# sailordiary/m3f.pytorch

Hardware: AMD Instinct MI355X
Metric: clips/sec (300-frame A+V, fwd+bwd) (higher is better)
Workload: dtype f32 (fp32-accurate products, fp32 accumulate: GEMMs as fp16x3 -- two fp16 terms per scaled operand, three MFMAs, error vs fp64 no larger than an fp32 GEMM's; the forward and backward recurrences at H=512 and H=256 as fp16x3 too (h is bounded; the backward producers split their values under a power-o

## Files before the change

### include/m3t_hip.h

```cpp
#ifndef M3T_HIP_H
#define M3T_HIP_H

#include <stddef.h>
#include <stdint.h>

#ifdef __cplusplus
extern "C" {
#endif

#define M3T_EINVAL 10001
#define M3T_MAX_SCANS 8
#define M3T_ESPIN 10002
#define M3T_SCAN_NO_PERSIST 1
#define M3T_SCAN_WHH 8
#define M3T_SCAN_FP32 4
#define M3T_SCAN_FAULT 16
#define M3T_SCAN_WIDE 32
#define M3T_BF16 2
#define M3T_GEMM_BACKGROUND 1
#define M3T_GEMM_BF16 2
#define M3T_GEMM_HIGH 256
#define M3T_GEMM_F16X3 1024
#define M3T_GEMM_BESIDE_SCAN 512
#define M3T_GEMM_EXCLUSIVE 8
// ... 105 lines not shown
    unsigned long long* amax;
    const float* wfrag;
} m3t_gru_bwd_desc;

size_t m3t_gru_bwd_prepare_floats(int H);
int m3t_gru_bwd_prepare(const float* const* w, int n, int H, int whh_direct, float* const* out, void* stream);

int m3t_gru_scan_workgroups(int n_scans, int H, int B, int T, int flags, int backward);
int m3t_gru_persist_count(void);
int m3t_gru_poll_error(void);
int m3t_gru_error_reset(void);
int m3t_gru_error_defer(int on);
int m3t_gru_inject_error(void* stream);
int m3t_gru_persist_owner(void);
int m3t_gru_scan_arena(void* arena, size_t bytes);
int m3t_gru_scan_arena_reset(void* arena);
int m3t_gru_scan_progress(unsigned* counters, int n_marks, const int* time_bounds, unsigned* need);
int m3t_gru_scan_progress_reset(unsigned* counters);
int m3t_gru_scan_progress_ok(int n_scans, int H, int B, int T, int flags, int backward);
int m3t_stream_wait_progress(const unsigned* counter, unsigned need, void* stream);
int m3t_gru_scan_after(void* event);
int m3t_gru_scan_events(void* start, void* end);
int m3t_gru_persist_profile(unsigned long long* out6);

int m3t_gru_scan_bwd(const m3t_gru_bwd_desc* scans, int n_scans, int B, int T,
                     float* ws, size_t ws_bytes, int flags, void* stream);

int m3t_att_fuse_fwd(const float* s_v, const float* s_a, const float* x_v, const float* x_a,
                     float* f, int rows, int D, void* stream);
int m3t_att_fuse_bwd(const float* df, const float* s_v, const float* s_a,
                     const float* x_v, const float* x_a,
                     float* ds_v, float* ds_a, float* dx_v, float* dx_a,
                     int rows, int D, void* stream);

int m3t_va_loss(const float* y_hat, int rows, int C, int iv, int ia,
                const float* valence, const float* arousal,
                const int64_t* class_expr, const uint8_t* expr_valid, int n_expr,
                float w_v, float w_a, float expr_w, int use_mse,
                float* out_scalars, float* dy, float* ws, size_t ws_bytes, void* stream);
size_t m3t_va_loss_ws_bytes(int rows);

size_t m3t_bn_cl_ws_bytes(size_t M, int C);
int m3t_bn_pool_cl_fwd(const float* x, size_t P, int H, int W, int C, int k, const float* gamma, const float* beta, float* run_mean, float* run_var,
                       float momentum, float eps, int training, float* yp, unsigned char* win, float* save_mean, float* save_invstd, float* ws,
                       size_t ws_bytes, void* stream);
int m3t_bn_pool_cl_bwd(const float* dyp, const float* x, const float* yp, const unsigned char* win, const float* gamma, const float* save_mean,
                       const float* save_invstd, size_t P, int H, int W, int C, int k, int training, float* dx, float* dgamma, float* dbeta,
                       float* dx_colsum, float* ws, size_t ws_bytes, void* stream);
int m3t_bn_cl_fwd(const float* x, size_t M, int C, const float* gamma, const float* beta, float* run_mean, float* run_var, float momentum,
                  float eps, int training, int relu, float* y, float* save_mean, float* save_invstd, float* ws, size_t ws_bytes, void* stream);
int m3t_bn_cl_bwd(const float* dy, const float* x, const float* y, const float* gamma, const float* save_mean, const float* save_invstd, size_t M,
                  int C, int training, int relu, float* dx, float* dgamma, float* dbeta, float* dx_colsum, float* ws, size_t ws_bytes, void* stream);
int m3t_pool_cl_fwd(const float* x, size_t P, int H, int W, int C, int kh, int kw, int sh, int sw, int ph, int pw, float* y, unsigned char* win,
                    void* stream);
int m3t_pool_cl_bwd(const float* dy, const unsigned char* win, size_t P, int H, int W, int C, int kh, int kw, int sh, int sw, int ph, int pw,
                    float* dx, void* stream);

int m3t_bn_add_relu_cl_fwd(const float* x, const float* shortcut, size_t M, int C, const float* gamma, const float* beta, float* run_mean,
                           float* run_var, float momentum, float eps, int training, float* y, float* save_mean, float* save_invstd, float* ws,
                           size_t ws_bytes, void* stream);
int m3t_bn_add_relu_cl_bwd(const float* dy, const float* x, const float* y, const float* gamma, const float* save_mean, const float* save_invstd,
                           size_t M, int C, int training, float* dx, float* ds, float* dgamma, float* dbeta, float* dx_colsum, float* ws,
                           size_t ws_bytes, void* stream);
int m3t_mean_cl_fwd(const float* x, size_t P, int HW, int C, float* y, void* stream);
int m3t_mean_cl_bwd(const float* dy, size_t P, int HW, int C, float* dx, void* stream);

// ... 260 lines not shown
```

### m3f.pytorch_amd/csrc/fuse_loss.hip

```cpp
#include "gru_common.h"
#include <cmath>
#include <cstdlib>
#include <mutex>

namespace {

__device__ __forceinline__ void fuse_weights(float sv, float sa, float& hv, float& ha, float& w0, float& w1) {
    hv = 1.f / (1.f + expf(-sv));
    ha = 1.f / (1.f + expf(-sa));
    const float m = fmaxf(hv, ha);
    const float ev = expf(hv - m), ea = expf(ha - m);
    const float inv = 1.f / (ev + ea);
    w0 = ev * inv;
    w1 = ea * inv;
}

__device__ __forceinline__ float mix2(float w0, float v, float w1, float a) { return fmaf(w0, v, w1 * a); }

__global__ __launch_bounds__(256) void att_fuse_fwd_kernel(const float* __restrict__ s_v, const float* __restrict__ s_a,
                                                           const float* __restrict__ x_v, const float* __restrict__ x_a,
                                                           float* __restrict__ f, int rows, int D, int vec) {
    const int lane = threadIdx.x & 63;
    const int row = blockIdx.x * 4 + (threadIdx.x >> 6);
    if (row >= rows) return;
// ... 23 lines not shown
    if (row >= rows) return;
    float hv, ha, w0, w1;
    fuse_weights(s_v[row], s_a[row], hv, ha, w0, w1);
    const size_t base = (size_t)row * D;
    float d0 = 0.f, d1 = 0.f;
    if (vec) {
        const float4* pg = reinterpret_cast<const float4*>(df + base);
        const float4* pv = reinterpret_cast<const float4*>(x_v + base);
        const float4* pa = reinterpret_cast<const float4*>(x_a + base);
        float4* qv = reinterpret_cast<float4*>(dx_v + base);
        float4* qa = reinterpret_cast<float4*>(dx_a + base);
        for (int i = lane; i < (D >> 2); i += 64) {
            const float4 g = pg[i], v = pv[i], a = pa[i];
            d0 += g.x * v.x + g.y * v.y + g.z * v.z + g.w * v.w;
            d1 += g.x * a.x + g.y * a.y + g.z * a.z + g.w * a.w;
            qv[i] = make_float4(w0 * g.x, w0 * g.y, w0 * g.z, w0 * g.w);
            qa[i] = make_float4(w1 * g.x, w1 * g.y, w1 * g.z, w1 * g.w);
        }
    } else {
        for (int i = lane; i < D; i += 64) {
            const float g = df[base + i];
            d0 += g * x_v[base + i];
            d1 += g * x_a[base + i];
            dx_v[base + i] = w0 * g;
            dx_a[base + i] = w1 * g;
        }
    }
    d0 = wave_sum(d0);
    d1 = wave_sum(d1);
    if (lane == 0) {
        const float dot = w0 * d0 + w1 * d1;
        ds_v[row] = w0 * (d0 - dot) * hv * (1.f - hv);
        ds_a[row] = w1 * (d1 - dot) * ha * (1.f - ha);
    }
}

__device__ __forceinline__ double wave_sum_d(double v) {
#pragma unroll
    for (int o = 32; o > 0; o >>= 1) v += __shfl_xor(v, o, 64);
    return v;
}
__device__ __forceinline__ double block_sum_d(double v, double* red) {
    const int lane = threadIdx.x & 63, w = threadIdx.x >> 6, nw = (blockDim.x + 63) >> 6;
    v = wave_sum_d(v);
    __syncthreads();
    if (lane == 0) red[w] = v;
    __syncthreads();
    double r = 0.0;
    for (int i = 0; i < nw; ++i) r += red[i];
    return r;
}

struct VaTerm { double mx, mt, ccc, mse, c1, c2, c3; };

__device__ __forceinline__ VaTerm va_term(double mx, double mt, double cov, double vsum, double mse, double invn, double nm1) {
    VaTerm s;
    const double den = vsum + (mx - mt) * (mx - mt);
    const double q = 2.0 * cov / (den * den);
    s.mx = mx; s.mt = mt; s.mse = mse;
    s.ccc = 2.0 * cov / den;
    s.c1 = 2.0 * invn / den;
    s.c2 = q * 2.0 * nm1;
    s.c3 = q * 2.0 * (mx - mt) * invn;
    return s;
}

// ... 387 lines not shown
extern "C" int m3t_sgd_step(float* p, const float* g, float* buf, size_t n, float lr, float momentum, float weight_decay,
                            int step, const float* guard, void* stream) {
    if (n == 0) return 0;
    if (!p || !g || !buf || step < 1) return M3T_EINVAL;
    int blocks = (int)((n + 255) / 256);
    if (blocks > 4096) blocks = 4096;
    sgd_kernel<<<blocks, 256, 0, (hipStream_t)stream>>>(p, g, buf, n, lr, momentum, weight_decay, step == 1, guard);
    M3T_LAUNCH_CHECK();
    return 0;
}

extern "C" int m3t_att_fuse_fwd(const float* s_v, const float* s_a, const float* x_v, const float* x_a, float* f,
                                int rows, int D, void* stream) {
    if (rows <= 0 || D <= 0) return 0;
    if (!s_v || !s_a || !x_v || !x_a || !f) return M3T_EINVAL;
    const int vec = (D % 4 == 0) && (((uintptr_t)x_v | (uintptr_t)x_a | (uintptr_t)f) % 16 == 0);
    att_fuse_fwd_kernel<<<cdiv(rows, 4), 256, 0, (hipStream_t)stream>>>(s_v, s_a, x_v, x_a, f, rows, D, vec);
    M3T_LAUNCH_CHECK();
    return 0;
}

extern "C" int m3t_att_fuse_bwd(const float* df, const float* s_v, const float* s_a, const float* x_v, const float* x_a,
                                float* ds_v, float* ds_a, float* dx_v, float* dx_a, int rows, int D, void* stream) {
    if (rows <= 0 || D <= 0) return 0;
    if (!df || !s_v || !s_a || !x_v || !x_a || !ds_v || !ds_a || !dx_v || !dx_a) return M3T_EINVAL;
    const int vec = (D % 4 == 0) &&
                    (((uintptr_t)x_v | (uintptr_t)x_a | (uintptr_t)df | (uintptr_t)dx_v | (uintptr_t)dx_a) % 16 == 0);
    att_fuse_bwd_kernel<<<cdiv(rows, 4), 256, 0, (hipStream_t)stream>>>(df, s_v, s_a, x_v, x_a, ds_v, ds_a, dx_v, dx_a,
                                                                         rows, D, vec);
    M3T_LAUNCH_CHECK();
    return 0;
}

extern "C" size_t m3t_va_loss_ws_bytes(int rows) { return rows > 0 ? (size_t)cdiv(rows, LB) * 16 * sizeof(double) : 0; }

extern "C" int m3t_va_loss(const float* y_hat, int rows, int C, int iv, int ia, const float* valence,
                           const float* arousal, const int64_t* class_expr, const uint8_t* expr_valid, int n_expr,
                           float w_v, float w_a, float expr_w, int use_mse, float* out_scalars, float* dy,
                           float* ws, size_t ws_bytes, void* stream) {
    if (rows <= 0 || C <= 0 || iv < 0 || ia < 0 || iv >= C || ia >= C || n_expr > C) return M3T_EINVAL;
    if (!y_hat || !valence || !arousal || !out_scalars || !dy) return M3T_EINVAL;
    if (n_expr > 0 && (!class_expr || !expr_valid)) return M3T_EINVAL;
    static const bool fused_on = !(getenv("M3T_VA_LOSS_FUSED") && getenv("M3T_VA_LOSS_FUSED")[0] == '0');
    const bool ws_ok = ws && ((uintptr_t)ws % 8) == 0 && ws_bytes >= m3t_va_loss_ws_bytes(rows);
    double* part = reinterpret_cast<double*>(ws);
    if (rows > 1024 && ws_ok && cdiv(rows, LB) <= 128 && fused_on) {
        VaSync* sync = va_sync_words();
        if (sync) {
            const int nb = cdiv(rows, LB);
            va_loss_fused_kernel<<<nb, LB, 0, (hipStream_t)stream>>>(y_hat, rows, C, iv, ia, valence, arousal, class_expr, expr_valid, n_expr, w_v,
                                                                     w_a, expr_w, use_mse, part, sync, 1 << 22, out_scalars, dy);
            M3T_LAUNCH_CHECK();
            return 0;
        }
    }
    if (rows > 1024 && ws_ok) {
        const int nb = cdiv(rows, LB);
        double* partA = part;
        double* partB = part + (size_t)nb * 8;
        hipStream_t s = (hipStream_t)stream;
        va_loss_sums_kernel<<<nb, LB, 0, s>>>(y_hat, rows, C, iv, ia, valence, arousal, class_expr, expr_valid, n_expr, partA);
        va_loss_moments_kernel<<<nb, LB, 0, s>>>(y_hat, rows, C, iv, ia, valence, arousal, partA, partB);
        va_loss_grad_kernel<<<nb, LB, 0, s>>>(y_hat, rows, C, iv, ia, valence, arousal, class_expr, expr_valid, n_expr, w_v, w_a,
                                             expr_w, use_mse, partA, partB, out_scalars, dy);
        M3T_LAUNCH_CHECK();
        return 0;
// ... 52 lines not shown
```

### m3f.pytorch_amd/csrc/gemm.hip

```cpp
#include "common.h"
#include <cstdio>
#include <cstdlib>

namespace {

constexpr int BM = 128, BN = 128, BK = 16, LDT = 132;

struct GemmParams {
    const float* A; const float* B; float* C; const float* bias; float* ws;
    int M, N, K, lda, ldb, ldc;
    int act, accumulate, splits, kchunk;
    int seg_len, seg_stride, a_off, b_off;
    int bf16;
    int vecA, vecB;
};

__device__ __forceinline__ int seg_row(int k, int seg_len, int seg_stride, int off) {
    return seg_len > 0 ? (k / seg_len) * seg_stride + (k % seg_len) + off : k;
}

__device__ __forceinline__ void load_kc(const float* __restrict__ src, int ld, int rows, int row0,
                                        int k0, int k_end, int vec, float4 (&r)[2]) {
    const int tid = threadIdx.x;
#pragma unroll
// ... 179 lines not shown
            acc[1][1] = __builtin_amdgcn_mfma_f32_32x32x2f32(fa[q][1], fb[q][1], acc[1][1], 0, 0, 0);
        }
        if (t + 1 < ntiles) sstore(cur ^ 1);
        __syncthreads();
    }

    const bool direct = p.splits == 1;
    float* dst = direct ? p.C : p.ws + (size_t)blockIdx.z * p.M * p.N;
    const int ldd = direct ? p.ldc : p.N;
#pragma unroll
    for (int i = 0; i < 2; ++i)
#pragma unroll
        for (int j = 0; j < 2; ++j) {
            const int col = bn + wn * 64 + j * 32 + l31;
            if (!FAST && col >= p.N) continue;
            const float bv = (direct && p.bias) ? p.bias[col] : 0.f;
#pragma unroll
            for (int r = 0; r < 16; ++r) {
                const int row = bm + wm * 64 + i * 32 + (r & 3) + 8 * (r >> 2) + 4 * hi;
                if (!FAST && row >= p.M) continue;
                float v = acc[i][j][r];
                float* q = dst + (size_t)row * ldd + col;
                if (direct) {
                    v += bv;
                    if (p.act == 1) v = m3t_relu(v);
                    if (p.accumulate) v += *q;
                }
                *q = v;
            }
        }
}

__global__ void splitk_reduce_kernel(const float* __restrict__ ws, float* __restrict__ C, const float* __restrict__ bias,
                                     int M, int N, int ldc, int splits, int act, int accumulate) {
    const size_t total = (size_t)M * N;
    for (size_t i = blockIdx.x * (size_t)blockDim.x + threadIdx.x; i < total; i += (size_t)gridDim.x * blockDim.x) {
        const int m = (int)(i / N), n = (int)(i % N);
        float s = 0.f;
        for (int k = 0; k < splits; ++k) s += ws[(size_t)k * total + i];
        if (bias) s += bias[n];
        if (act == 1) s = m3t_relu(s);
        float* q = C + (size_t)m * ldc + n;
        if (accumulate) s += *q;
        *q = s;
    }
}

constexpr int SK_FOLD = 32;
__global__ __launch_bounds__(256) void splitk_fold4_kernel(float* __restrict__ ws, size_t total4, int splits) {
    float4* w4 = reinterpret_cast<float4*>(ws);
    const int k0 = blockIdx.y * SK_FOLD, k1 = min(splits, k0 + SK_FOLD);
    for (size_t i = blockIdx.x * (size_t)blockDim.x + threadIdx.x; i < total4; i += (size_t)gridDim.x * blockDim.x) {
        float4 s = make_float4(0.f, 0.f, 0.f, 0.f);
        int k = k0;
        for (; k + 8 <= k1; k += 8) {
            float4 v[8];
#pragma unroll
            for (int u = 0; u < 8; ++u) v[u] = w4[(size_t)(k + u) * total4 + i];
#pragma unroll
            for (int u = 0; u < 8; ++u) { s.x += v[u].x; s.y += v[u].y; s.z += v[u].z; s.w += v[u].w; }
        }
        for (; k < k1; ++k) {
            const float4 v = w4[(size_t)k * total4 + i];
            s.x += v.x; s.y += v.y; s.z += v.z; s.w += v.w;
        }
        w4[(size_t)k0 * total4 + i] = s;
    }
}

__global__ __launch_bounds__(256) void splitk_reduce4_kernel(const float* __restrict__ ws, float* __restrict__ C,
                                                             const float* __restrict__ bias, int M, int N, int ldc, int splits,
                                                             int act, int accumulate, int kstride) {
    const size_t total4 = (size_t)M * N / 4, slab4 = total4 * (size_t)kstride;
    const float4* w4 = reinterpret_cast<const float4*>(ws);
    const int n4 = N / 4;
    for (size_t i = blockIdx.x * (size_t)blockDim.x + threadIdx.x; i < total4; i += (size_t)gridDim.x * blockDim.x) {
        float4 s = make_float4(0.f, 0.f, 0.f, 0.f);
        int k = 0;
        for (; k + 8 <= splits; k += 8) {
            float4 v[8];
#pragma unroll
            for (int u = 0; u < 8; ++u) v[u] = w4[(size_t)(k + u) * slab4 + i];
#pragma unroll
            for (int u = 0; u < 8; ++u) { s.x += v[u].x; s.y += v[u].y; s.z += v[u].z; s.w += v[u].w; }
        }
        for (; k < splits; ++k) {
            const float4 v = w4[(size_t)k * slab4 + i];
            s.x += v.x; s.y += v.y; s.z += v.z; s.w += v.w;
        }
        const int m = (int)(i / n4), n = (int)(i % n4) * 4;
        if (bias) { s.x += bias[n]; s.y += bias[n + 1]; s.z += bias[n + 2]; s.w += bias[n + 3]; }
        if (act == 1) { s.x = m3t_relu(s.x); s.y = m3t_relu(s.y); s.z = m3t_relu(s.z); s.w = m3t_relu(s.w); }
        float4* q = reinterpret_cast<float4*>(C + (size_t)m * ldc + n);
        if (accumulate) { const float4 c = *q; s.x += c.x; s.y += c.y; s.z += c.z; s.w += c.w; }
        *q = s;
    }
}


constexpr int ABSMAX_REGIONS = 16;
struct AbsmaxArgs { M3TRegion r[ABSMAX_REGIONS]; };
__global__ __launch_bounds__(256) void f16x3_absmax_kernel(AbsmaxArgs a, unsigned epoch) {
    const M3TRegion r = a.r[blockIdx.y];
    const unsigned long long total = r.rows * (unsigned long long)r.c4;
    if ((unsigned long long)blockIdx.x * 256 >= total && blockIdx.x > 0) return;
    unsigned m = 0u;
    const bool dense = (unsigned long long)r.c4 * 4ull == r.ld;
    auto at = [&](unsigned long long i) -> const uint4* {
        if (dense) return reinterpret_cast<const uint4*>(r.p + (size_t)i * 4);
        const unsigned long long row = i / (unsigned)r.c4;
        return reinterpret_cast<const uint4*>(r.p + (size_t)(row * r.ld + (i - row * (unsigned)r.c4) * 4ull));
    };
    auto fin = [](unsigned b) { b &= 0x7fffffffu; return b < 0x7f800000u ? b : 0u; };
    auto fold = [&](const uint4& v) { m = max(max(m, fin(v.x)), max(fin(v.y), max(fin(v.z), fin(v.w)))); };
    const unsigned long long stride = (unsigned long long)gridDim.x * 256;
    unsigned long long i = (unsigned long long)blockIdx.x * 256 + threadIdx.x;
    for (; i + 3 * stride < total; i += 4 * stride) {
        const uint4 v0 = *at(i), v1 = *at(i + stride), v2 = *at(i + 2 * stride), v3 = *at(i + 3 * stride);
        fold(v0); fold(v1); fold(v2); fold(v3);
    }
    for (; i < total; i += stride) fold(*at(i));
#pragma unroll
    for (int o = 32; o > 0; o >>= 1) m = max(m, (unsigned)__shfl_xor((int)m, o, 64));
    __shared__ unsigned red[4];
    if ((threadIdx.x & 63) == 0) red[threadIdx.x >> 6] = m;
    __syncthreads();
    if (threadIdx.x == 0) {
        m = max(max(red[0], red[1]), max(red[2], red[3]));
        const unsigned long long val = ((unsigned long long)epoch << 32) | m;
        if (__hip_atomic_load(r.slot, __ATOMIC_RELAXED, __HIP_MEMORY_SCOPE_AGENT) < val) atomicMax(r.slot, val);
    }
}

static int launch_absmax(const M3TRegion* regs, int n, unsigned epoch, hipStream_t s) {
    AbsmaxArgs a;
    unsigned long long tm = 0;
    for (int i = 0; i < n; ++i) {
        a.r[i] = regs[i];
        const unsigned long long t = regs[i].rows * (unsigned long long)regs[i].c4;
        if (t > tm) tm = t;
    }
    for (int i = n; i < ABSMAX_REGIONS; ++i) a.r[i] = regs[0];
    unsigned long long blocks = (tm + 256ull * 8 - 1) / (256ull * 8);
    static int total = 0;
    if (!total) { const char* e = getenv("M3T_ABSMAX_TOTAL"); total = (e && atoi(e) > 0) ? atoi(e) : 384; }
    const unsigned long long cap = (unsigned long long)max(16, total / max(1, n));
    if (blocks > cap) blocks = cap;
    if (blocks < 1) blocks = 1;
    if (blocks > 1024) blocks = 1024;
    f16x3_absmax_kernel<<<dim3((unsigned)blocks, n), 256, 0, s>>>(a, epoch);
    return (int)hipGetLastError();
}

static void launch_splitk_reduce(const float* ws, float* C, const float* bias, int M, int N, int ldc, int splits, int act,
                                 int accumulate, hipStream_t s) {
    const size_t total = (size_t)M * N;
    if (N % 4 == 0 && ldc % 4 == 0 && ((uintptr_t)C % 16) == 0 && ((uintptr_t)ws % 16) == 0) {
        int blocks = (int)((total / 4 + 255) / 256);
        if (blocks > 4096) blocks = 4096;
        if (splits >= 4 * SK_FOLD && blocks <= 64) {
            const int groups = (splits + SK_FOLD - 1) / SK_FOLD;
            splitk_fold4_kernel<<<dim3(blocks, groups), 256, 0, s>>>(const_cast<float*>(ws), total / 4, splits);
            splitk_reduce4_kernel<<<blocks, 256, 0, s>>>(ws, C, bias, M, N, ldc, groups, act, accumulate, SK_FOLD);
            return;
        }
        splitk_reduce4_kernel<<<blocks, 256, 0, s>>>(ws, C, bias, M, N, ldc, splits, act, accumulate, 1);
        return;
    }
    int blocks = (int)((total + 255) / 256);
    if (blocks > 2048) blocks = 2048;
    splitk_reduce_kernel<<<blocks, 256, 0, s>>>(ws, C, bias, M, N, ldc, splits, act, accumulate);
}

__global__ void colsum_kernel(const float* __restrict__ X, int M, int N, int ld, float* __restrict__ out, int accumulate) {
    __shared__ float red[8][33];
    const int c = blockIdx.x * 32 + (threadIdx.x & 31);
    const int rl = threadIdx.x >> 5;
    float s = 0.f;
    if (c < N)
        for (int m = rl; m < M; m += 8) s += X[(size_t)m * ld + c];
    red[rl][threadIdx.x & 31] = s;
    __syncthreads();
    if (rl == 0 && c < N) {
        float t = 0.f;
#pragma unroll
        for (int i = 0; i < 8; ++i) t += red[i][threadIdx.x & 31];
        out[c] = accumulate ? out[c] + t : t;
    }
}

__global__ void colsum_partial_kernel(const float* __restrict__ X, int M, int N, int ld, float* __restrict__ part, int rows_per) {
    __shared__ float red[8][33];
    const int c = blockIdx.x * 32 + (threadIdx.x & 31);
    const int rl = threadIdx.x >> 5;
    const int m0 = blockIdx.y * rows_per, m1 = min(M, m0 + rows_per);
    float s = 0.f;
    if (c < N)
        for (int m = m0 + rl; m < m1; m += 8) s += X[(size_t)m * ld + c];
    red[rl][threadIdx.x & 31] = s;
    __syncthreads();
    if (rl == 0 && c < N) {
        float t = 0.f;
#pragma unroll
        for (int i = 0; i < 8; ++i) t += red[i][threadIdx.x & 31];
// ... 107 lines not shown
        sl.dev = it->second.dev;
    }
    M3TRegion regs[2];
    int n = 0;
    if (!have_a) { regs[n] = ra; regs[n].slot = sl.dev; *use_a = sl.dev; ++n; }
    if (!have_b) { regs[n] = rb; regs[n].slot = sl.dev + 1; *use_b = sl.dev + 1; ++n; }
    return launch_absmax(regs, n, sl.epoch, s);
}

int m3t_absmax_regions(const M3TRegion* regs, int n, hipStream_t s) {
    for (int i = 0; i < n; i += ABSMAX_REGIONS) {
        const int rc = launch_absmax(regs + i, n - i < ABSMAX_REGIONS ? n - i : ABSMAX_REGIONS, 0u, s);
        if (rc) return rc;
    }
    return 0;
}

extern "C" int m3t_absmax(int n, const float* const* x, const size_t* rows, const int* cols, const size_t* ld,
                          unsigned long long* const* slots, void* stream) {
    if (n <= 0) return 0;
    if (n > ABSMAX_REGIONS || !x || !rows || !cols || !ld || !slots) return M3T_EINVAL;
    M3TRegion regs[ABSMAX_REGIONS];
    for (int i = 0; i < n; ++i) {
        if (!x[i] || !slots[i] || cols[i] <= 0 || cols[i] % 4 != 0 || ld[i] % 4 != 0 || (uintptr_t)x[i] % 16 != 0 || (uintptr_t)slots[i] % 8 != 0)
            return M3T_EINVAL;
        regs[i] = M3TRegion{x[i], (unsigned long long)rows[i], (unsigned long long)ld[i], cols[i] / 4, slots[i]};
    }
    return launch_absmax(regs, n, 0u, (hipStream_t)stream);
}

int m3t_sgemm_x6_launch(int transA, int transB, int M, int N, int K, const float* A, int lda, const float* B, int ldb,
                        float* C, int ldc, const float* bias, int act, int accumulate, int seg_len, int seg_stride,
                        int a_off, int b_off, float* ws, int splits, int kchunk, size_t dyn_lds, int bf16_operands, int narrow,
                        const unsigned long long* amax_a, const unsigned long long* amax_b, hipStream_t s);

int m3t_sgemm_x6d_launch(int transA, int transB, int M, int N, int K, const float* A, int lda, const float* B, int ldb,
                         float* C, int ldc, const float* bias, int act, int accumulate, int seg_len, int seg_stride,
                         int a_off, int b_off, float* ws, int splits, int kchunk, int bf16_operands,
                         const unsigned long long* amax_a, const unsigned long long* amax_b, hipStream_t s);

int m3t_sgemm_x6w_launch(int transA, int transB, int M, int N, int K, const float* A, int lda, const float* B, int ldb,
                         float* C, int ldc, const float* bias, int act, int accumulate, int seg_len, int seg_stride,
                         int a_off, int b_off, float* ws, int splits, int kchunk, int bf16_operands,
                         const unsigned long long* amax_a, const unsigned long long* amax_b, hipStream_t s);

static int x6d_mode() { return 2; }

bool m3t_f16x3_enabled() {
    static int on = -1;
    if (on < 0) {
        const char* e = getenv("M3T_GEMM_F16X3");
        on = (e && e[0] == '0') ? 0 : 1;
    }
    return on == 1;
}

bool m3t_gemm_tr_enabled() {
    static int on = -1;
    if (on < 0) {
        const char* e = getenv("M3T_GEMM_TR");
        on = (e && e[0] == '0') ? 0 : 1;
    }
    return on == 1;
}

static bool f16x3_on_x6d() { return true; }

static bool x6_enabled() {
    static int on = -1;
    if (on < 0) {
        const char* e = getenv("M3T_GEMM_X6");
        on = (e && e[0] == '0') ? 0 : 1;
    }
    return on == 1;
}

constexpr int GEMM_NO_WIDE = 1 << 20;
// ... 32 lines not shown
    };
    if (ws_bytes && K >= 512) {
        for (int sp = 1; sp <= 96 && sp <= K / 96 && (sp == 1 || (size_t)sp <= cap); ++sp) {
            const double t = model(tiles, ns_per_k, sp);
            if (t < best) { best = t; splits = sp; }
        }
    } else best = model(tiles, ns_per_k, 1);
    g.wide = 0;
    if (x6 && !bf16 && !high && N % 256 == 0 && x6w_enabled() && !(flags & (M3T_GEMM_BACKGROUND | GEMM_NO_WIDE))) {
        const int tiles_w = cdiv(M, BM) * (N / 256);
        double best_w = 1e30; int splits_w = 1;
        if (ws_bytes && K >= 512) {
            for (int sp = 1; sp <= 96 && sp <= K / 96 && (sp == 1 || (size_t)sp <= cap); ++sp) {
                const double t = model(tiles_w, 2.0 * 0.8 * ns_per_k, sp);
                if (t < best_w) { best_w = t; splits_w = sp; }
            }
        } else best_w = model(tiles_w, 2.0 * 0.8 * ns_per_k, 1);
        if (best_w < best) { g.wide = 1; splits = splits_w; }
    }
    int kchunk = cdiv(cdiv(K, splits), kq) * kq;
    if (kchunk < kq) kchunk = kq;
    g.kernel = x6 ? 1 : 0; g.kchunk = kchunk; g.splits = K > 0 ? cdiv(K, kchunk) : 1;
    g.narrow = (!g.wide && x6 && narrow_mode() && (n64 || narrow_mode() == 2 || (g.splits == 1 && tiles <= 384))) ? 1 : 0;
    return g;
}

extern "C" int m3t_sgemm_plan(int transA, int M, int N, int K, int seg_len, size_t ws_bytes, int flags, int* kernel, int* splits) {
    if (M <= 0 || N <= 0 || K < 0 || !kernel || !splits) return M3T_EINVAL;
    const GemmPlan g = plan_gemm(transA, M, N, K, seg_len, true, ws_bytes, flags | (transA ? GEMM_NO_WIDE : 0));
    *kernel = g.kernel; *splits = g.splits;
    return 0;
}

extern "C" int m3t_sgemm(int transA, int transB, int M, int N, int K, const float* A, int lda, const float* B, int ldb,
                         float* C, int ldc, const float* bias, int act, int accumulate, int seg_len, int seg_stride,
                         int a_off, int b_off, float* ws, size_t ws_bytes, int flags, void* stream) {
    return m3t_sgemm_scaled(transA, transB, M, N, K, A, lda, B, ldb, C, ldc, bias, act, accumulate, seg_len, seg_stride, a_off, b_off,
                            ws, ws_bytes, flags, nullptr, nullptr, stream);
}

extern "C" int m3t_sgemm_scaled(int transA, int transB, int M, int N, int K, const float* A, int lda, const float* B, int ldb,
                                float* C, int ldc, const float* bias, int act, int accumulate, int seg_len, int seg_stride,
                                int a_off, int b_off, float* ws, size_t ws_bytes, int flags, const unsigned long long* amax_a,
                                const unsigned long long* amax_b, void* stream) {
    if (M <= 0 || N <= 0) return 0;
    if (K < 0 || !A || !B || !C) return M3T_EINVAL;
    if (seg_len > 0 && !(transA == 1 && transB == 0)) return M3T_EINVAL;
    GemmParams p;
    p.A = A; p.B = B; p.C = C; p.bias = bias; p.ws = ws;
    p.M = M; p.N = N; p.K = K; p.lda = lda; p.ldb = ldb; p.ldc = ldc;
    p.act = act; p.accumulate = accumulate;
    p.seg_len = seg_len; p.seg_stride = seg_stride; p.a_off = a_off; p.b_off = b_off;
    p.bf16 = (flags & M3T_GEMM_BF16) ? 1 : 0;
    p.vecA = (lda % 4 == 0) && ((uintptr_t)A % 16 == 0);
    p.vecB = (ldb % 4 == 0) && ((uintptr_t)B % 16 == 0);
    const int tm = cdiv(M, BM), tn = cdiv(N, BN);
    const GemmPlan g = plan_gemm(transA, M, N, K, seg_len, p.vecA && p.vecB, ws ? ws_bytes : 0,
                                 flags | ((transA == 0 && transB == 1) ? 0 : GEMM_NO_WIDE));
    int splits = g.splits, kchunk = g.kchunk;
    {
        static int beside_wgs = -1;
        if (beside_wgs < 0) { const char* e = getenv("M3T_GEMM_BESIDE_WGS"); beside_wgs = e ? atoi(e) : 384; }
        if (beside_wgs > 0 && (flags & M3T_GEMM_BESIDE_SCAN) && g.kernel != 0 && !g.wide && g.splits > 1) {
            const int tiles = cdiv(M, BM) * cdiv(N, g.narrow ? 64 : BN);
            int sp = (beside_wgs + tiles / 2) / tiles;
            if (sp < 1) sp = 1;
            if (sp < g.splits) {
                kchunk = cdiv(cdiv(K, sp), 32) * 32;
                splits = cdiv(K, kchunk);
            }
        }
    }
    p.splits = splits; p.kchunk = kchunk;
    hipStream_t s = (hipStream_t)stream;
    if (g.kernel != 0) {
        int rc;
        const int f16x3 = (!p.bf16 && !(flags & M3T_GEMM_HIGH) && (flags & M3T_GEMM_F16X3) && m3t_f16x3_enabled()) ? 1 : 0;
        const bool wide_tr = f16x3 && !g.wide && !g.narrow && !(transA == 0 && transB == 1) && !(flags & M3T_GEMM_BACKGROUND) && N % 256 == 0 &&
                             K % 32 == 0 && x6w_enabled() && m3t_gemm_tr_enabled() && tr_wide_wins(flags);
        const unsigned long long* use_a = nullptr; const unsigned long long* use_b = nullptr;
        if (f16x3) {
            const size_t kr = seg_len > 0 ? (size_t)(K / seg_len - 1) * seg_stride + seg_len : (size_t)K;
            const float* A0 = seg_len > 0 ? A + (size_t)a_off * lda : A;
            const float* B0 = seg_len > 0 ? B + (size_t)b_off * ldb : B;
            const M3TRegion ra{A0, (unsigned long long)(transA ? kr : (size_t)M), (unsigned long long)lda, (transA ? M : K) / 4, nullptr};
            const M3TRegion rb{B0, (unsigned long long)(transB ? (size_t)N : kr), (unsigned long long)ldb, (transB ? K : N) / 4, nullptr};
            const int rm = m3t_f16x3_measure(ra, amax_a, rb, amax_b, &use_a, &use_b, s);
            if (rm) return rm;
        }
        if (g.wide || wide_tr)
            rc = m3t_sgemm_x6w_launch(transA, transB, M, N, K, A, lda, B, ldb, C, ldc, bias, act, accumulate, seg_len, seg_stride,
                                      a_off, b_off, ws, splits, kchunk, f16x3 ? 3 : 0, use_a, use_b, s);
        else if (!g.narrow && K % 32 == 0 && (!f16x3 || f16x3_on_x6d()) && !(flags & (M3T_GEMM_BACKGROUND | M3T_GEMM_HIGH)) && (x6d_mode() == 1 || (x6d_mode() == 2 && !(flags & M3T_GEMM_BESIDE_SCAN))))
            rc = m3t_sgemm_x6d_launch(transA, transB, M, N, K, A, lda, B, ldb, C, ldc, bias, act, accumulate, seg_len, seg_stride,
                                      a_off, b_off, ws, splits, kchunk, p.bf16 ? 1 : ((flags & M3T_GEMM_HIGH) ? 2 : (f16x3 ? 3 : 0)), use_a, use_b, s);
        else
            rc = m3t_sgemm_x6_launch(transA, transB, M, N, K, A, lda, B, ldb, C, ldc, bias, act, accumulate, seg_len, seg_stride,
                                     a_off, b_off, ws, splits, kchunk, (flags & M3T_GEMM_BACKGROUND) ? (size_t)40 * 1024 : 0,
                                     p.bf16 ? 1 : ((flags & M3T_GEMM_HIGH) ? 2 : (f16x3 ? 3 : 0)), g.narrow, use_a, use_b, s);
        if (rc) return rc;
        if (splits > 1) {
            launch_splitk_reduce(ws, C, bias, M, N, ldc, splits, act, accumulate, s);
            M3T_LAUNCH_CHECK();
        }
        return 0;
    }
    dim3 grid(tn, tm, splits), block(256);
    const bool fast = (M % BM == 0) && (N % BN == 0) && (K % BK == 0) && K > 0 && p.vecA && p.vecB;
    const size_t dyn = (flags & M3T_GEMM_BACKGROUND) ? (size_t)56 * 1024 + 0 : 0;
#define M3T_GEMM_LAUNCH(TA_, TB_)                                                 \
    do {                                                                          \
        if (fast && seg_len >= BK) sgemm_kernel<TA_, TB_, true, true><<<grid, block, dyn, s>>>(p); \
        else if (seg_len > 0) sgemm_kernel<TA_, TB_, false><<<grid, block, dyn, s>>>(p);           \
        else if (fast) sgemm_kernel<TA_, TB_, true><<<grid, block, dyn, s>>>(p);    \
        else sgemm_kernel<TA_, TB_, false><<<grid, block, dyn, s>>>(p);             \
    } while (0)
    if (transA == 0 && transB == 1) M3T_GEMM_LAUNCH(0, 1);
    else if (transA == 0 && transB == 0) M3T_GEMM_LAUNCH(0, 0);
    else if (transA == 1 && transB == 0) M3T_GEMM_LAUNCH(1, 0);
    else M3T_GEMM_LAUNCH(1, 1);
#undef M3T_GEMM_LAUNCH
    M3T_LAUNCH_CHECK();
    if (splits > 1) {
        launch_splitk_reduce(ws, C, bias, M, N, ldc, splits, act, accumulate, s);
        M3T_LAUNCH_CHECK();
    }
    return 0;
}

int m3t_sgemm_x6_window_launch(int n, const m3t_window_problem* pr, int transB, int M, int N, int K, int lda, int ldb, int ldc,
                               int act, int mw_len, int mw_stride, int mw_off, int f16x3, int narrow, hipStream_t s);

extern "C" int m3t_sgemm_window_batch(int n, const m3t_window_problem* pr, int transB, int n_seg, int win_len, int win_stride, int win_off,
                                      int N, int K, int lda, int ldb, int ldc, int act, int flags, void* stream) {
    if (n <= 0 || n_seg <= 0 || win_len <= 0 || N <= 0) return 0;
    if (n > M3T_WINDOW_BATCH || !pr || K <= 0 || win_stride < win_len || win_off < 0 || win_off + win_len > win_stride) return M3T_EINVAL;
    const long long Ml = (long long)n_seg * win_len;
    if (Ml > 0x7fffffffll || (long long)n_seg * win_stride > 0x7fffffffll) return M3T_EINVAL;
    const int M = (int)Ml;
    if (!x6_enabled() || M % 128 != 0 || N % 64 != 0 || K % 32 != 0 || lda % 4 != 0 || ldb % 4 != 0 || (flags & (M3T_GEMM_BF16 | M3T_GEMM_HIGH)))
        return M3T_EINVAL;
    const int f16x3 = ((flags & M3T_GEMM_F16X3) && m3t_f16x3_enabled()) ? 1 : 0;
    hipStream_t s = (hipStream_t)stream;
    m3t_window_problem use[M3T_WINDOW_BATCH];
    for (int i = 0; i < n; ++i) {
        use[i] = pr[i];
        if (!use[i].A || !use[i].B || !use[i].C || (uintptr_t)use[i].A % 16 != 0 || (uintptr_t)use[i].B % 16 != 0) return M3T_EINVAL;
        if (f16x3 && (!use[i].amax_a || !use[i].amax_b)) {
            if (n > 1) return M3T_EINVAL;
            const size_t span = (size_t)(n_seg - 1) * win_stride + win_len;
            const M3TRegion ra{use[i].A + (size_t)win_off * lda, (unsigned long long)span, (unsigned long long)lda, K / 4, nullptr};
            const M3TRegion rb{use[i].B, (unsigned long long)(transB ? (size_t)N : (size_t)K), (unsigned long long)ldb, (transB ? K : N) / 4, nullptr};
            const int rm = m3t_f16x3_measure(ra, use[i].amax_a, rb, use[i].amax_b, &use[i].amax_a, &use[i].amax_b, s);
            if (rm) return rm;
        }
    }
    const int narrow = (N % 128 != 0 || (long long)(M / 128) * (N / 128) * n <= 384) ? 1 : 0;
    return m3t_sgemm_x6_window_launch(n, use, transB ? 1 : 0, M, N, K, lda, ldb, ldc, act, win_len, win_stride, win_off, f16x3, narrow, s);
}

extern "C" int m3t_sgemm_window(int transB, int n_seg, int win_len, int win_stride, int win_off, int N, int K,
                                const float* A, int lda, const float* B, int ldb, float* C, int ldc, const float* bias,
                                int act, int accumulate, int flags, const unsigned long long* amax_a, const unsigned long long* amax_b,
                                void* stream) {
    const m3t_window_problem pr{A, B, C, bias, amax_a, amax_b, accumulate};
    return m3t_sgemm_window_batch(1, &pr, transB, n_seg, win_len, win_stride, win_off, N, K, lda, ldb, ldc, act, flags, stream);
}
// ... 45 lines not shown
        *reinterpret_cast<float4*>(out + r * ldo + 4 * (size_t)c) = o;
    }
}
__global__ __launch_bounds__(256) void f16x3_split_perm_kernel(const float* __restrict__ w, float* __restrict__ out, size_t R, int T, int Cc, size_t sR,
                                                               size_t sT, size_t sC, const unsigned long long* __restrict__ slot) {
    float sc, inv;
    m3t_f16_scale((unsigned)*slot, sc, inv);
    const int c4 = Cc >> 2;
    const size_t total = R * (size_t)T * c4;
    for (size_t i = blockIdx.x * (size_t)blockDim.x + threadIdx.x; i < total; i += (size_t)gridDim.x * blockDim.x) {
        const int c = (int)(i % (size_t)c4);
        const size_t rt = i / (size_t)c4;
        const int t = (int)(rt % (size_t)T);
        const size_t r = rt / (size_t)T;
        const float* q = w + r * sR + (size_t)t * sT + (size_t)(4 * c) * sC;
        const sp_f32x2 a = (sp_f32x2){q[0], q[sC]} * sc, b = (sp_f32x2){q[2 * sC], q[3 * sC]} * sc;
        const sp_f16x2 ha = __builtin_convertvector(a, sp_f16x2), hb = __builtin_convertvector(b, sp_f16x2);
        const sp_f16x2 la = __builtin_convertvector(a - __builtin_convertvector(ha, sp_f32x2), sp_f16x2);
        const sp_f16x2 lb = __builtin_convertvector(b - __builtin_convertvector(hb, sp_f32x2), sp_f16x2);
        float4 o;
        o.x = __uint_as_float(__builtin_bit_cast(unsigned, ha)); o.y = __uint_as_float(__builtin_bit_cast(unsigned, hb));
        o.z = __uint_as_float(__builtin_bit_cast(unsigned, la)); o.w = __uint_as_float(__builtin_bit_cast(unsigned, lb));
        *reinterpret_cast<float4*>(out + (r * T + t) * (size_t)Cc + 4 * (size_t)c) = o;
    }
}
}

int m3t_sgemm_x6_pre_launch(int M, int N, int K, const float* A, int lda, const float* B, int ldb, float* C, int ldc, const float* bias,
                            int act, int accumulate, int narrow, const unsigned long long* amax_a, const unsigned long long* amax_b, hipStream_t s);

extern "C" int m3t_sgemm_pre(int M, int N, int K, const float* A_img, int lda, const float* B_img, int ldb, float* C, int ldc,
                             const float* bias, int act, int accumulate, const unsigned long long* amax_a, const unsigned long long* amax_b,
                             void* stream) {
    if (M <= 0 || N <= 0) return 0;
    if (!A_img || !B_img || !C || !amax_a || !amax_b || K <= 0 || !x6_enabled() || !m3t_f16x3_enabled() || M % 128 != 0 || N % 64 != 0 ||
        K % 32 != 0 || lda % 4 != 0 || ldb % 4 != 0 || (uintptr_t)A_img % 16 != 0 || (uintptr_t)B_img % 16 != 0)
        return M3T_EINVAL;
    const int narrow = (N % 128 != 0 || (long long)(M / 128) * (N / 128) <= 384) ? 1 : 0;
    return m3t_sgemm_x6_pre_launch(M, N, K, A_img, lda, B_img, ldb, C, ldc, bias, act, accumulate, narrow, amax_a, amax_b, (hipStream_t)stream);
}

namespace {
__global__ __launch_bounds__(256) void f16x3_image_b_kernel(const float* __restrict__ w, unsigned char* __restrict__ img, int N, int K8, size_t ld,
                                                            const unsigned long long* __restrict__ slot) {
    float sc, inv;
    m3t_f16_scale((unsigned)*slot, sc, inv);
    const size_t total = (size_t)N * K8;
    for (size_t i = blockIdx.x * (size_t)blockDim.x + threadIdx.x; i < total; i += (size_t)gridDim.x * blockDim.x) {
        const int r = (int)(i % 64); const size_t q = i / 64;
        const int o = (int)(q % K8); const int rb = (int)(q / K8);
        const float* src = w + ((size_t)rb * 64 + r) * ld + 8 * (size_t)o;
        const float4 v0 = *reinterpret_cast<const float4*>(src), v1 = *reinterpret_cast<const float4*>(src + 4);
        const float x[8] = {v0.x, v0.y, v0.z, v0.w, v1.x, v1.y, v1.z, v1.w};
        unsigned hi[4], lo[4];
#pragma unroll
        for (int e = 0; e < 4; ++e) {
            const sp_f32x2 a = (sp_f32x2){x[2 * e], x[2 * e + 1]} * sc;
            const sp_f16x2 h = __builtin_convertvector(a, sp_f16x2);
            const sp_f16x2 l = __builtin_convertvector(a - __builtin_convertvector(h, sp_f32x2), sp_f16x2);
            hi[e] = __builtin_bit_cast(unsigned, h); lo[e] = __builtin_bit_cast(unsigned, l);
        }
        unsigned char* dst = img + (((size_t)rb * K8 + o) * 2) * 1024 + (size_t)r * 16;
        *reinterpret_cast<uint4*>(dst) = make_uint4(hi[0], hi[1], hi[2], hi[3]);
        *reinterpret_cast<uint4*>(dst + 1024) = make_uint4(lo[0], lo[1], lo[2], lo[3]);
    }
}
}

int m3t_sgemm_x6w_bimg_launch(int M, int N, int K, const float* A, int lda, const float* B_img, float* C, int ldc, const float* bias, int act,
                              int accumulate, float* ws, int splits, int kchunk, const unsigned long long* amax_a,
                              const unsigned long long* amax_b, hipStream_t s);

extern "C" int m3t_f16x3_image_b(const float* w, int N, int K, size_t ld, float* img, const unsigned long long* slot, void* stream) {
    if (N <= 0 || K <= 0) return 0;
    if (!w || !img || !slot || N % 64 != 0 || K % 8 != 0 || ld % 4 != 0 || (uintptr_t)w % 16 != 0 || (uintptr_t)img % 16 != 0) return M3T_EINVAL;
    const size_t total = (size_t)N * (K / 8);
    size_t blocks = (total + 255) / 256;
    if (blocks > 4096) blocks = 4096;
    f16x3_image_b_kernel<<<(unsigned)blocks, 256, 0, (hipStream_t)stream>>>(w, reinterpret_cast<unsigned char*>(img), N, K / 8, ld, slot);
    M3T_LAUNCH_CHECK();
    return 0;
}

extern "C" int m3t_sgemm_bimg(int M, int N, int K, const float* A, int lda, const float* B_img, float* C, int ldc, const float* bias, int act,
                              int accumulate, float* ws, size_t ws_bytes, const unsigned long long* amax_a, const unsigned long long* amax_b,
                              void* stream) {
    if (M <= 0 || N <= 0) return 0;
    if (!A || !B_img || !C || !amax_b || K <= 0 || !x6_enabled() || !m3t_f16x3_enabled() || M % 128 != 0 || N % 256 != 0 || K % 32 != 0 ||
        lda % 4 != 0 || (uintptr_t)A % 16 != 0 || (uintptr_t)B_img % 16 != 0)
        return M3T_EINVAL;
    hipStream_t s = (hipStream_t)stream;
    const unsigned long long* use_a = amax_a; const unsigned long long* use_b = amax_b;
    if (!amax_a) {
        const M3TRegion ra{A, (unsigned long long)M, (unsigned long long)lda, K / 4, nullptr};
        const M3TRegion rb{A, 0ull, 0ull, 0, nullptr};
        const int rm = m3t_f16x3_measure(ra, nullptr, rb, amax_b, &use_a, &use_b, s);
        if (rm) return rm;
    }
    const GemmPlan g = plan_gemm(0, M, N, K, 0, true, ws ? ws_bytes : 0, M3T_GEMM_F16X3);
    const int splits = g.wide ? g.splits : 1, kchunk = g.wide ? g.kchunk : K;
    const int rc = m3t_sgemm_x6w_bimg_launch(M, N, K, A, lda, B_img, C, ldc, bias, act, accumulate, ws, splits, kchunk, use_a, use_b, s);
    if (rc) return rc;
    if (splits > 1) { launch_splitk_reduce(ws, C, bias, M, N, ldc, splits, act, accumulate, s); M3T_LAUNCH_CHECK(); }
    return 0;
}

int m3t_sgemm_ring_launch(int transA, int transB, int M, int N, int K, const float* A, int lda, const float* B, int ldb, float* C, int ldc,
                          const float* bias, int act, int accumulate, int seg_len, int seg_stride, int a_off, int b_off, float* ws, int splits,
                          int kchunk, const unsigned long long* amax_a, const unsigned long long* amax_b, int variant, hipStream_t s);

extern "C" int m3t_sgemm_ring(int transA, int transB, int M, int N, int K, const float* A, int lda, const float* B, int ldb, float* C, int ldc,
                              const float* bias, int act, int accumulate, int seg_len, int seg_stride, int a_off, int b_off, float* ws,
                              size_t ws_bytes, int splits, const unsigned long long* amax_a, const unsigned long long* amax_b, int variant,
                              void* stream) {
    if (M <= 0 || N <= 0) return 0;
    if (!A || !B || !C || K <= 0 || !m3t_f16x3_enabled() || N % 256 != 0 || K % 16 != 0 || lda % 4 != 0 || ldb % 4 != 0 ||
        (uintptr_t)A % 16 != 0 || (uintptr_t)B % 16 != 0 || splits < 1)
        return M3T_EINVAL;
    if ((transA == 1 && transB == 1) || (transA == 1 && M % 4 != 0)) return M3T_EINVAL;
    if (seg_len > 0 && !(transA == 1 && transB == 0 && seg_len >= 32 && K % seg_len == 0)) return M3T_EINVAL;
    if ((variant < 0 || variant > 3) && !getenv("M3T_RING_ABLATIONS")) return M3T_EINVAL;
    hipStream_t s = (hipStream_t)stream;
    const unsigned long long* use_a = amax_a; const unsigned long long* use_b = amax_b;
    if (!amax_a || !amax_b) {
        const size_t kr = seg_len > 0 ? (size_t)(K / seg_len - 1) * seg_stride + seg_len : (size_t)K;
        const float* A0 = seg_len > 0 ? A + (size_t)a_off * lda : A;
        const float* B0 = seg_len > 0 ? B + (size_t)b_off * ldb : B;
        const M3TRegion ra{A0, (unsigned long long)(transA ? kr : (size_t)M), (unsigned long long)lda, (transA ? M : K) / 4, nullptr};
        const M3TRegion rb{B0, (unsigned long long)(transB ? (size_t)N : kr), (unsigned long long)ldb, (transB ? K : N) / 4, nullptr};
        const int rm = m3t_f16x3_measure(ra, amax_a, rb, amax_b, &use_a, &use_b, s);
        if (rm) return rm;
    }
    int kchunk = cdiv(cdiv(K, splits), 32) * 32;
    splits = cdiv(K, kchunk);
    if (splits > 1 && (!ws || ws_bytes < (size_t)splits * M * N * sizeof(float))) return M3T_EINVAL;
    const int rc = m3t_sgemm_ring_launch(transA, transB, M, N, K, A, lda, B, ldb, C, ldc, bias, act, accumulate, seg_len, seg_stride, a_off, b_off,
                                         ws, splits, kchunk, use_a, use_b, variant, s);
    if (rc) return rc;
    if (splits > 1) { launch_splitk_reduce(ws, C, bias, M, N, ldc, splits, act, accumulate, s); M3T_LAUNCH_CHECK(); }
    return 0;
}

extern "C" int m3t_f16x3_split_perm(const float* w, size_t R, int T, int Cc, size_t sR, size_t sT, size_t sC, float* out,
                                    const unsigned long long* slot, void* stream) {
    if (R == 0 || T <= 0 || Cc <= 0) return 0;
    if (!w || !out || !slot || Cc % 4 != 0 || (uintptr_t)out % 16 != 0) return M3T_EINVAL;
    const size_t total = R * (size_t)T * (Cc / 4);
    int blocks = (int)((total + 255) / 256 > 4096 ? 4096 : (total + 255) / 256);
    f16x3_split_perm_kernel<<<blocks, 256, 0, (hipStream_t)stream>>>(w, out, R, T, Cc, sR, sT, sC, slot);
    M3T_LAUNCH_CHECK();
    return 0;
}

extern "C" int m3t_f16x3_split(const float* x, size_t rows, int cols, size_t ld, float* out, size_t ldo, const unsigned long long* slot,
                               void* stream) {
    if (rows == 0 || cols <= 0) return 0;
    if (!x || !out || !slot || cols % 4 != 0 || ld % 4 != 0 || ldo % 4 != 0 || (uintptr_t)x % 16 != 0 || (uintptr_t)out % 16 != 0) return M3T_EINVAL;
    const size_t total = rows * (size_t)(cols / 4);
    int blocks = (int)((total + 255) / 256 > 8192 ? 8192 : (total + 255) / 256);
    f16x3_split_kernel<<<blocks, 256, 0, (hipStream_t)stream>>>(x, out, rows, cols / 4, ld, ldo, slot);
    M3T_LAUNCH_CHECK();
    return 0;
}

extern "C" int m3t_conv3d_taps(const float* src, const float* w_taps, float* dst, int N, int C_src, int C_dst, int T, int H, int W,
                               int To, int Ho, int Wo, int kt, int kh, int kw, int base_t, int base_h, int base_w, int sign, int flags,
                               const unsigned long long* amax_src, const unsigned long long* amax_w, float* ws, size_t ws_bytes, float* dst_planes,
                               void* stream) {
    if (N <= 0 || C_dst <= 0) return 0;
    if (!src || !w_taps || !dst || C_src <= 0 || T <= 0 || H <= 0 || W <= 0 || To <= 0 || Ho <= 0 || Wo <= 0 || kt <= 0 || kh <= 0 || kw <= 0 ||
        (sign != 1 && sign != -1))
        return M3T_EINVAL;
// ... 241 lines not shown
```

### m3f.pytorch_amd/csrc/gemm_x6.hip

```cpp
#include "common.h"
#include <cstdlib>

namespace {

typedef __bf16 bf16x8 __attribute__((ext_vector_type(8)));
typedef __bf16 bf16x4 __attribute__((ext_vector_type(4)));

constexpr int XM = 128, XN = 128, XK = 32;
constexpr int PLANE = XM * 16 + 64;
constexpr int SPLIT_BYTES = 4 * PLANE;
constexpr int OPER_BYTES = 3 * SPLIT_BYTES;
constexpr int TRROW = XM * 2 + 64;
constexpr int TRTERM = XK * TRROW;
static_assert(2 * TRTERM <= OPER_BYTES, "the transposed-read image must fit the operand's LDS");
typedef short s16x4 __attribute__((ext_vector_type(4)));

struct X6Params {
    const float* A; const float* B; float* C; const float* bias; float* ws;
    int M, N, K, lda, ldb, ldc;
    int act, accumulate, splits, kchunk;
    int seg_len, seg_stride, a_off, b_off;
    int cv_T, cv_C, cv_K, cv_dil, cv_lead, cv_anti;
    size_t cv_btap;
    const float* cv_mask; const float* cv_res; float* cv_pre;
// ... 451 lines not shown
    float vmax = 0.f;
#pragma unroll
    for (int i = 0; i < 2; ++i)
#pragma unroll
        for (int j = 0; j < NJ; ++j) {
            const int col = bn + wn * 32 * NJ + j * 32 + l31;
            const float bv = (direct && p.bias) ? p.bias[col] : 0.f;
            float dm[4] = {1.f, 1.f, 1.f, 1.f};
#pragma unroll
            for (int r = 0; r < 16; ++r) {
                const int row = bm + wm * 64 + i * 32 + (r & 3) + 8 * (r >> 2) + 4 * hi;
                if (C3ROWS && row >= p.M) continue;
                if (CONV && p.cv_drop.on && (r & 3) == 0) m3t_drop_mask4(p.cv_drop, (uint32_t)row >> 2, (uint32_t)col, dm);
                float v = acc[i][j][r];
                if (NS == 4) v = v * sc_ia * sc_ib;
                float* q = dst + (size_t)(MW ? rowmap[row - bm] : row) * ldd + col;
                if (CONV) {
                    const size_t o = (size_t)row * ldd + col;
                    v += bv;
                    if (p.cv_pre) p.cv_pre[o] = v;
                    const float mk = p.cv_drop.on ? dm[r & 3] : (p.cv_mask ? p.cv_mask[o] : 1.f);
                    if (p.act == 1) v = m3t_relu(v) * mk;
                    else if (p.act == 2) v = m3t_relu(m3t_relu(v) * mk + p.cv_res[o]);
                    else if (p.cv_res) v += p.cv_res[o];
                    vmax = fmaxf(vmax, m3t_fin_abs(v));
                } else if (direct) {
                    v += bv;
                    if (p.act == 1) v = m3t_relu(v);
                    if (p.accumulate) v += *q;
                }
                *q = v;
            }
        }
    if (CONV && p.cv_amax) {
        __shared__ float red4[4];
        m3t_block_raise_slot(p.cv_amax, vmax, red4);
    }
}

const X6Batch g_no_batch = {};

}

int m3t_sgemm_x6_launch(int transA, int transB, int M, int N, int K, const float* A, int lda, const float* B, int ldb,
                        float* C, int ldc, const float* bias, int act, int accumulate, int seg_len, int seg_stride,
                        int a_off, int b_off, float* ws, int splits, int kchunk, size_t dyn_lds, int bf16_operands, int narrow,
                        const unsigned long long* amax_a, const unsigned long long* amax_b, hipStream_t s) {
    X6Params p;
    p.amax_a = amax_a; p.amax_b = amax_b;
    p.A = A; p.B = B; p.C = C; p.bias = bias; p.ws = ws;
    p.M = M; p.N = N; p.K = K; p.lda = lda; p.ldb = ldb; p.ldc = ldc;
    p.act = act; p.accumulate = accumulate; p.splits = splits; p.kchunk = kchunk;
    p.seg_len = seg_len; p.seg_stride = seg_stride; p.a_off = a_off; p.b_off = b_off;
    p.cv_T = p.cv_C = p.cv_K = p.cv_dil = p.cv_lead = p.cv_anti = 0; p.cv_btap = 0; p.cv_mask = p.cv_res = nullptr; p.cv_pre = nullptr;
    p.cv_drop = m3t_make_drop(0.f, 0ull);
    p.cv_amax = nullptr;
    p.mw_len = p.mw_stride = p.mw_off = 0;
    p.c3_T = p.c3_H = p.c3_W = p.c3_To = p.c3_Ho = p.c3_Wo = p.c3_kt = p.c3_kh = p.c3_kw = p.c3_bt = p.c3_bh = p.c3_bw = p.c3_sg = p.c3_C = 0; p.c3_st = p.c3_sh = p.c3_sw = 1; p.tr_S = 0;
    dim3 grid(N / (narrow ? 64 : XN), M / XM, splits), block(256);
#define M3T_X6_DISPATCH(NS_, XNT_, TR_)                                                                                                                 \
    do {                                                                                                                                               \
        if (seg_len > 0) sgemm_x6_kernel<1, 0, true, NS_, false, XNT_, false, 0, 0, TR_><<<grid, block, dyn_lds, s>>>(p, g_no_batch);                  \
        else if (transA == 0 && transB == 1) sgemm_x6_kernel<0, 1, false, NS_, false, XNT_><<<grid, block, dyn_lds, s>>>(p, g_no_batch);               \
        else if (transA == 0 && transB == 0) sgemm_x6_kernel<0, 0, false, NS_, false, XNT_, false, 0, 0, TR_><<<grid, block, dyn_lds, s>>>(p, g_no_batch); \
        else if (transA == 1 && transB == 0) sgemm_x6_kernel<1, 0, false, NS_, false, XNT_, false, 0, 0, TR_><<<grid, block, dyn_lds, s>>>(p, g_no_batch); \
        else sgemm_x6_kernel<1, 1, false, NS_, false, XNT_, false, 0, 0, TR_><<<grid, block, dyn_lds, s>>>(p, g_no_batch);                             \
    } while (0)
    if (bf16_operands == 3 && (!amax_a || !amax_b)) return M3T_EINVAL;
    const bool tr = m3t_gemm_tr_enabled();
    if (bf16_operands == 1) { if (narrow) M3T_X6_DISPATCH(1, 64, false); else M3T_X6_DISPATCH(1, 128, false); }
    else if (bf16_operands == 2) { if (narrow) M3T_X6_DISPATCH(2, 64, false); else M3T_X6_DISPATCH(2, 128, false); }
    else if (bf16_operands == 3 && tr) { if (narrow) M3T_X6_DISPATCH(4, 64, true); else M3T_X6_DISPATCH(4, 128, true); }
    else if (bf16_operands == 3) { if (narrow) M3T_X6_DISPATCH(4, 64, false); else M3T_X6_DISPATCH(4, 128, false); }
    else { if (narrow) M3T_X6_DISPATCH(3, 64, false); else M3T_X6_DISPATCH(3, 128, false); }
#undef M3T_X6_DISPATCH
    hipError_t e = hipGetLastError();
    return (int)e;
}

int m3t_sgemm_x6_window_launch(int n, const m3t_window_problem* pr, int transB, int M, int N, int K, int lda, int ldb, int ldc,
                               int act, int mw_len, int mw_stride, int mw_off, int f16x3, int narrow, hipStream_t s) {
    X6Params p;
    X6Batch bt = {};
    for (int i = 0; i < n; ++i) {
        if (f16x3 && (!pr[i].amax_a || !pr[i].amax_b)) return M3T_EINVAL;
        bt.A[i] = pr[i].A; bt.B[i] = pr[i].B; bt.C[i] = pr[i].C; bt.bias[i] = pr[i].bias;
        bt.amax_a[i] = pr[i].amax_a; bt.amax_b[i] = pr[i].amax_b; bt.accumulate[i] = pr[i].accumulate;
    }
    p.amax_a = p.amax_b = nullptr;
// ... 177 lines not shown
```

### m3f.pytorch_amd/csrc/gemm_x6d.hip

```cpp
#include "common.h"
#include <cstdlib>
#include <type_traits>

namespace {

typedef __bf16 bf16x8 __attribute__((ext_vector_type(8)));
typedef __bf16 bf16x4 __attribute__((ext_vector_type(4)));
typedef __bf16 bf16x2 __attribute__((ext_vector_type(2)));
typedef float f32x2 __attribute__((ext_vector_type(2)));
typedef unsigned u32x2 __attribute__((ext_vector_type(2)));
typedef unsigned u32x4 __attribute__((ext_vector_type(4)));
typedef float f32x4 __attribute__((ext_vector_type(4)));

constexpr int BM = 128, BN = 128, BKS = 16, NTH = 256;
constexpr int PLANEB = BM * 16 + 128;
constexpr int SPLITB = 2 * PLANEB;
constexpr int OPERB = 3 * SPLITB;
constexpr int STAGEB = 2 * OPERB;
constexpr int TRROW = BM * 2 + 64;
constexpr int TRTERM = BKS * TRROW;
static_assert(2 * TRTERM <= OPERB, "the transposed-read image must fit the operand's LDS");
typedef short s16x4 __attribute__((ext_vector_type(4)));
typedef short s16x8 __attribute__((ext_vector_type(8)));

struct X6DParams {
    const float* A; const float* B; float* C; const float* bias; float* ws;
    int M, N, K, lda, ldb, ldc;
    int act, accumulate, splits, kchunk;
    int seg_len, seg_stride, a_off, b_off;
    int cv_T, cv_C, cv_K, cv_dil, cv_lead, cv_anti;
    size_t cv_btap;
    const float* cv_mask; const float* cv_res; float* cv_pre;
    M3TDrop cv_drop;
    const unsigned long long* amax_a;
    const unsigned long long* amax_b;
};

typedef _Float16 f16x2 __attribute__((ext_vector_type(2)));
typedef _Float16 f16x8 __attribute__((ext_vector_type(8)));
constexpr int planes_of(int NS) { return NS == 4 ? 2 : NS; }
template <int NS>
__device__ __forceinline__ void split3_pair(f32x2 v, unsigned (&o)[3], float scale = 1.f) {
    if (NS == 4) {
        const f32x2 vs = v * scale;
        const f16x2 h = __builtin_convertvector(vs, f16x2);
        o[0] = __builtin_bit_cast(unsigned, h);
        const f32x2 r1 = vs - __builtin_convertvector(h, f32x2);
        const f16x2 l = __builtin_convertvector(r1, f16x2);
        o[1] = __builtin_bit_cast(unsigned, l);
        return;
    }
    const bf16x2 h = __builtin_convertvector(v, bf16x2);
    o[0] = __builtin_bit_cast(unsigned, h);
    if (NS == 1) return;
    f32x2 hf;
    hf.x = __uint_as_float(o[0] << 16); hf.y = __uint_as_float(o[0] & 0xffff0000u);
    const f32x2 r1 = v - hf;
    const bf16x2 m = __builtin_convertvector(r1, bf16x2);
    o[1] = __builtin_bit_cast(unsigned, m);
    if (NS == 2) return;
    f32x2 mf;
    mf.x = __uint_as_float(o[1] << 16); mf.y = __uint_as_float(o[1] & 0xffff0000u);
    const f32x2 r2 = r1 - mf;
    const bf16x2 l = __builtin_convertvector(r2, bf16x2);
    o[2] = __builtin_bit_cast(unsigned, l);
}

template <int NS>
// ... 229 lines not shown
    const bool direct = p.splits == 1;
    float* dst = direct ? p.C : p.ws + (size_t)blockIdx.z * p.M * p.N;
    const int ldd = direct ? p.ldc : p.N;
#pragma unroll
    for (int i = 0; i < 2; ++i)
#pragma unroll
        for (int j = 0; j < 2; ++j) {
            const int col = bn + wn * 64 + j * 32 + l31;
            const float bv = (direct && p.bias) ? p.bias[col] : 0.f;
            float dm[4] = {1.f, 1.f, 1.f, 1.f};
#pragma unroll
            for (int r = 0; r < 16; ++r) {
                const int row = bm + wm * 64 + i * 32 + (r & 3) + 8 * (r >> 2) + 4 * hi;
                if (CONV && p.cv_drop.on && (r & 3) == 0) m3t_drop_mask4(p.cv_drop, (uint32_t)row >> 2, (uint32_t)col, dm);
                float v = acc[i][j][r];
                if (NS == 4) v = v * sc_ia * sc_ib;
                float* q = dst + (size_t)row * ldd + col;
                if (CONV) {
                    const size_t o = (size_t)row * ldd + col;
                    v += bv;
                    if (p.cv_pre) p.cv_pre[o] = v;
                    const float mk = p.cv_drop.on ? dm[r & 3] : (p.cv_mask ? p.cv_mask[o] : 1.f);
                    if (p.act == 1) v = m3t_relu(v) * mk;
                    else if (p.act == 2) v = m3t_relu(m3t_relu(v) * mk + p.cv_res[o]);
                    else if (p.cv_res) v += p.cv_res[o];
                } else if (direct) {
                    v += bv;
                    if (p.act == 1) v = m3t_relu(v);
                    if (p.accumulate) v += *q;
                }
                *q = v;
            }
        }
}

}

int m3t_sgemm_x6d_launch(int transA, int transB, int M, int N, int K, const float* A, int lda, const float* B, int ldb,
                         float* C, int ldc, const float* bias, int act, int accumulate, int seg_len, int seg_stride,
                         int a_off, int b_off, float* ws, int splits, int kchunk, int bf16_operands,
                         const unsigned long long* amax_a, const unsigned long long* amax_b, hipStream_t s) {
    X6DParams p;
    p.amax_a = amax_a; p.amax_b = amax_b;
    if (bf16_operands == 3 && (!amax_a || !amax_b)) return M3T_EINVAL;
    p.A = A; p.B = B; p.C = C; p.bias = bias; p.ws = ws;
    p.M = M; p.N = N; p.K = K; p.lda = lda; p.ldb = ldb; p.ldc = ldc;
    p.act = act; p.accumulate = accumulate; p.splits = splits; p.kchunk = kchunk;
    p.seg_len = seg_len; p.seg_stride = seg_stride; p.a_off = a_off; p.b_off = b_off;
    p.cv_T = p.cv_C = p.cv_K = p.cv_dil = p.cv_lead = p.cv_anti = 0; p.cv_btap = 0; p.cv_mask = p.cv_res = nullptr; p.cv_pre = nullptr;
    p.cv_drop = m3t_make_drop(0.f, 0ull);
    dim3 grid(N / BN, M / BM, splits), block(NTH);
    const size_t lds = 2 * (size_t)STAGEB;
    const bool tr = m3t_gemm_tr_enabled();
#define M3T_X6D_GO(TA_, TB_, SEG_, NS_, TR_)                                                                          \
    do {                                                                                                               \
        static bool attr_set = false;                                                                                  \
        if (!attr_set) {                                                                                               \
            hipError_t ea = hipFuncSetAttribute((const void*)sgemm_x6d_kernel<TA_, TB_, SEG_, NS_, false, TR_>,        \
                                                hipFuncAttributeMaxDynamicSharedMemorySize, (int)lds);                \
            if (ea != hipSuccess) return (int)ea;                                                                      \
            attr_set = true;                                                                                           \
        }                                                                                                              \
        sgemm_x6d_kernel<TA_, TB_, SEG_, NS_, false, TR_><<<grid, block, lds, s>>>(p);                                 \
    } while (0)
#define M3T_X6D_DISPATCH(NS_, TR_)                                                                                   \
    do {                                                                                                               \
        if (seg_len > 0) M3T_X6D_GO(1, 0, true, NS_, TR_);                                                             \
        else if (transA == 0 && transB == 1) M3T_X6D_GO(0, 1, false, NS_, false);                                      \
        else if (transA == 0 && transB == 0) M3T_X6D_GO(0, 0, false, NS_, TR_);                                        \
        else if (transA == 1 && transB == 0) M3T_X6D_GO(1, 0, false, NS_, TR_);                                        \
        else M3T_X6D_GO(1, 1, false, NS_, TR_);                                                                        \
    } while (0)
    if (bf16_operands == 1) M3T_X6D_DISPATCH(1, false);
    else if (bf16_operands == 2) M3T_X6D_DISPATCH(2, false);
    else if (bf16_operands == 3) { if (tr) M3T_X6D_DISPATCH(4, true); else M3T_X6D_DISPATCH(4, false); }
    else M3T_X6D_DISPATCH(3, false);
#undef M3T_X6D_DISPATCH
#undef M3T_X6D_GO
    return (int)hipGetLastError();
}


int m3t_conv_x6d_launch(const float* x, const float* w_t, const float* bias, const float* res, const float* mask, float* y,
                        float* pre, int B, int T, int Ci, int Co, int K, int dil, int lead, int act, int anti, int bf16_operands,
                        M3TDrop drop, hipStream_t s) {
    X6DParams p;
    p.amax_a = p.amax_b = nullptr;
    p.A = x; p.B = w_t; p.C = y; p.bias = bias; p.ws = nullptr;
    p.M = B * T; p.N = Co; p.K = K * Ci; p.lda = Ci; p.ldb = anti ? Co : Ci; p.ldc = Co;
    p.act = act; p.accumulate = 0; p.splits = 1; p.kchunk = K * Ci;
    p.seg_len = p.seg_stride = p.a_off = p.b_off = 0;
    p.cv_T = T; p.cv_C = Ci; p.cv_K = K; p.cv_dil = dil; p.cv_lead = lead; p.cv_anti = anti;
    p.cv_btap = (size_t)Co * Ci; p.cv_mask = mask; p.cv_res = res; p.cv_pre = pre; p.cv_drop = drop;
    dim3 grid(Co / BN, p.M / BM, 1), block(NTH);
    const size_t lds = 2 * (size_t)STAGEB;
#define M3T_CONVD_GO(TB_, NS_)                                                                                            \
    do {                                                                                                                   \
        static bool attr_set = false;                                                                                      \
        if (!attr_set) {                                                                                                   \
            hipError_t ea = hipFuncSetAttribute((const void*)sgemm_x6d_kernel<0, TB_, false, NS_, true>,                   \
                                                hipFuncAttributeMaxDynamicSharedMemorySize, (int)lds);                    \
            if (ea != hipSuccess) return (int)ea;                                                                          \
            attr_set = true;                                                                                               \
        }                                                                                                                  \
        sgemm_x6d_kernel<0, TB_, false, NS_, true><<<grid, block, lds, s>>>(p);                                            \
    } while (0)
    if (anti) {
        if (bf16_operands == 1) M3T_CONVD_GO(0, 1); else if (bf16_operands == 2) M3T_CONVD_GO(0, 2); else M3T_CONVD_GO(0, 3);
    } else {
        if (bf16_operands == 1) M3T_CONVD_GO(1, 1); else if (bf16_operands == 2) M3T_CONVD_GO(1, 2); else M3T_CONVD_GO(1, 3);
    }
#undef M3T_CONVD_GO
    return (int)hipGetLastError();
}
```

### m3f.pytorch_amd/csrc/gemm_x6w.hip

```cpp
#include "common.h"
#include <atomic>
#include <cstdlib>

namespace {

typedef __bf16 bf16x8 __attribute__((ext_vector_type(8)));
typedef __bf16 bf16x2 __attribute__((ext_vector_type(2)));
typedef float f32x2 __attribute__((ext_vector_type(2)));
typedef unsigned u32x2 __attribute__((ext_vector_type(2)));
typedef unsigned u32x4 __attribute__((ext_vector_type(4)));
typedef float f32x4 __attribute__((ext_vector_type(4)));
typedef _Float16 f16x2 __attribute__((ext_vector_type(2)));
typedef _Float16 f16x8 __attribute__((ext_vector_type(8)));

constexpr int WM = 128, WN = 256, WKS = 16, WTH = 256;
constexpr int PLA = WM * 16 + 128;
constexpr int PLB = WN * 16 + 128;
constexpr int planes_of(int NS) { return NS == 4 ? 2 : NS; }
constexpr int opera(int NS) { return planes_of(NS) * 2 * PLA; }
constexpr int operb(int NS) { return planes_of(NS) * 2 * PLB; }
constexpr int stageb(int NS) { return opera(NS) + operb(NS); }
constexpr int TRROWA = WM * 2 + 64, TRROWB = WN * 2 + 64;
constexpr int opera_of(int NS, bool tr) { return tr ? 2 * WKS * TRROWA : opera(NS); }
constexpr int operb_of(int NS, bool tr) { return tr ? 2 * WKS * TRROWB : operb(NS); }
constexpr int stageb_of(int NS, int TA, int TB, bool tr) { return opera_of(NS, tr && TA == 1) + operb_of(NS, tr && TB == 0); }
typedef short s16x4 __attribute__((ext_vector_type(4)));

struct X6WParams {
    const float* A; const float* B; float* C; const float* bias; float* ws;
    int M, N, K, lda, ldb, ldc;
    int act, accumulate, splits, kchunk;
    int seg_len, seg_stride, a_off, b_off;
    const unsigned long long* amax_a;
    const unsigned long long* amax_b;
};

template <int NS>
__device__ __forceinline__ void split3_pair(f32x2 v, unsigned (&o)[3], float scale = 1.f) {
    if (NS == 4) {
        const f32x2 vs = v * scale;
        const f16x2 h = __builtin_convertvector(vs, f16x2);
        o[0] = __builtin_bit_cast(unsigned, h);
        const f32x2 r1 = vs - __builtin_convertvector(h, f32x2);
        const f16x2 l = __builtin_convertvector(r1, f16x2);
        o[1] = __builtin_bit_cast(unsigned, l);
        return;
    }
    const bf16x2 h = __builtin_convertvector(v, bf16x2);
    o[0] = __builtin_bit_cast(unsigned, h);
    f32x2 hf;
    hf.x = __uint_as_float(o[0] << 16); hf.y = __uint_as_float(o[0] & 0xffff0000u);
    const f32x2 r1 = v - hf;
    const bf16x2 m = __builtin_convertvector(r1, bf16x2);
    o[1] = __builtin_bit_cast(unsigned, m);
    f32x2 mf;
    mf.x = __uint_as_float(o[1] << 16); mf.y = __uint_as_float(o[1] & 0xffff0000u);
    const f32x2 r2 = r1 - mf;
    const bf16x2 l = __builtin_convertvector(r2, bf16x2);
    o[2] = __builtin_bit_cast(unsigned, l);
}

template <int NS, int NR, int PL>
__device__ __forceinline__ void kc_store_w(unsigned char* __restrict__ S, const f32x4 (&r)[NR], float scale) {
    const int tid = threadIdx.x;
    unsigned char* q = S + ((tid >> 1) & 1) * PL + (tid >> 2) * 16 + (tid & 1) * 8;
#pragma unroll
    for (int i = 0; i < NR; ++i) {
// ... 246 lines not shown
    for (int t = 0; t < nst; t += 2) {
        gload(ra0, rb0);
        stage(buf0, buf1, ra1, rb1);
        asm volatile("s_waitcnt lgkmcnt(0)\n\ts_barrier" ::: "memory");
        gload(ra1, rb1);
        stage(buf1, buf0, ra0, rb0);
        asm volatile("s_waitcnt lgkmcnt(0)\n\ts_barrier" ::: "memory");
    }
    }

    const bool direct = p.splits == 1;
    float* dst = direct ? p.C : p.ws + (size_t)blockIdx.z * p.M * p.N;
    const int ldd = direct ? p.ldc : p.N;
#pragma unroll
    for (int i = 0; i < 2; ++i)
#pragma unroll
        for (int j = 0; j < 4; ++j) {
            const int col = bn + wn * 128 + j * 32 + l31;
            const float bv = (direct && p.bias) ? p.bias[col] : 0.f;
#pragma unroll
            for (int r = 0; r < 16; ++r) {
                const int row = bm + wm * 64 + i * 32 + (r & 3) + 8 * (r >> 2) + 4 * hi;
                float v = acc[i][j][r];
                if (NS == 4) v = v * sc_ia * sc_ib;
                float* q = dst + (size_t)row * ldd + col;
                if (direct) {
                    v += bv;
                    if (p.act == 1) v = m3t_relu(v);
                    if (p.accumulate) v += *q;
                }
                *q = v;
            }
        }
}

}

int m3t_sgemm_x6w_launch(int transA, int transB, int M, int N, int K, const float* A, int lda, const float* B, int ldb,
                         float* C, int ldc, const float* bias, int act, int accumulate, int seg_len, int seg_stride,
                         int a_off, int b_off, float* ws, int splits, int kchunk, int bf16_operands,
                         const unsigned long long* amax_a, const unsigned long long* amax_b, hipStream_t s) {
    if (bf16_operands != 0 && bf16_operands != 3) return M3T_EINVAL;
    if (bf16_operands == 3 && (!amax_a || !amax_b)) return M3T_EINVAL;
    X6WParams p;
    p.amax_a = amax_a; p.amax_b = amax_b;
    p.A = A; p.B = B; p.C = C; p.bias = bias; p.ws = ws;
    p.M = M; p.N = N; p.K = K; p.lda = lda; p.ldb = ldb; p.ldc = ldc;
    p.act = act; p.accumulate = accumulate; p.splits = splits; p.kchunk = kchunk;
    p.seg_len = seg_len; p.seg_stride = seg_stride; p.a_off = a_off; p.b_off = b_off;
    dim3 grid(N / WN, M / WM, splits), block(WTH);
    int dev = 0;
    if (hipGetDevice(&dev) != hipSuccess || dev < 0 || dev >= 32) return M3T_EINVAL;
#define M3T_X6W_GO(TA_, TB_, SEG_, NS_, TR_)                                                                          \
    do {                                                                                                               \
        const size_t lds = 2 * (size_t)stageb_of(NS_, TA_, TB_, TR_);                                                  \
        static std::atomic<unsigned> attr_set{0};                      \
        if (!(attr_set.load(std::memory_order_relaxed) & (1u << dev))) {                                               \
            hipError_t ea = hipFuncSetAttribute((const void*)sgemm_x6w_kernel<TA_, TB_, SEG_, NS_, 0, TR_>,            \
                                                hipFuncAttributeMaxDynamicSharedMemorySize, (int)lds);                \
            if (ea != hipSuccess) return (int)ea;                                                                      \
            attr_set.fetch_or(1u << dev, std::memory_order_relaxed);                                                   \
        }                                                                                                              \
        sgemm_x6w_kernel<TA_, TB_, SEG_, NS_, 0, TR_><<<grid, block, lds, s>>>(p);                                     \
    } while (0)
#define M3T_X6W_DISPATCH(NS_, TR_)                                                                                   \
    do {                                                                                                               \
        if (seg_len > 0) M3T_X6W_GO(1, 0, true, NS_, TR_);                                                             \
        else if (transA == 0 && transB == 1) M3T_X6W_GO(0, 1, false, NS_, false);                                      \
        else if (transA == 0 && transB == 0) M3T_X6W_GO(0, 0, false, NS_, TR_);                                        \
        else if (transA == 1 && transB == 0) M3T_X6W_GO(1, 0, false, NS_, TR_);                                        \
        else M3T_X6W_GO(1, 1, false, NS_, TR_);                                                                        \
    } while (0)
    if (bf16_operands == 3 && m3t_gemm_tr_enabled()) M3T_X6W_DISPATCH(4, true);
    else if (bf16_operands == 3) M3T_X6W_DISPATCH(4, false);
    else M3T_X6W_DISPATCH(3, false);
#undef M3T_X6W_DISPATCH
#undef M3T_X6W_GO
    return (int)hipGetLastError();
}

int m3t_sgemm_x6w_bimg_launch(int M, int N, int K, const float* A, int lda, const float* B_img, float* C, int ldc, const float* bias, int act,
                              int accumulate, float* ws, int splits, int kchunk, const unsigned long long* amax_a,
                              const unsigned long long* amax_b, hipStream_t s) {
    if (!amax_a || !amax_b) return M3T_EINVAL;
    X6WParams p;
    p.amax_a = amax_a; p.amax_b = amax_b;
    p.A = A; p.B = B_img; p.C = C; p.bias = bias; p.ws = ws;
    p.M = M; p.N = N; p.K = K; p.lda = lda; p.ldb = 0; p.ldc = ldc;
    p.act = act; p.accumulate = accumulate; p.splits = splits; p.kchunk = kchunk;
    p.seg_len = p.seg_stride = p.a_off = p.b_off = 0;
    dim3 grid(N / WN, M / WM, splits), block(WTH);
    const size_t lds = 2 * (size_t)stageb(4);
    int dev = 0;
    if (hipGetDevice(&dev) != hipSuccess || dev < 0 || dev >= 32) return M3T_EINVAL;
    static std::atomic<unsigned> attr_set{0};
    if (!(attr_set.load(std::memory_order_relaxed) & (1u << dev))) {
        hipError_t ea = hipFuncSetAttribute((const void*)sgemm_x6w_kernel<0, 1, false, 4, 1>, hipFuncAttributeMaxDynamicSharedMemorySize, (int)lds);
        if (ea != hipSuccess) return (int)ea;
        attr_set.fetch_or(1u << dev, std::memory_order_relaxed);
    }
    sgemm_x6w_kernel<0, 1, false, 4, 1><<<grid, block, lds, s>>>(p);
    return (int)hipGetLastError();
}
```

### m3f.pytorch_amd/m3t/_lib.py

```python
import ctypes as C
import os

_HERE = os.path.dirname(os.path.abspath(__file__))
LIB_PATH = os.environ.get("M3T_LIB_PATH") or os.path.join(os.path.dirname(_HERE), "lib", "libm3t_hip.so")
CSRC_DIR = os.path.join(os.path.dirname(_HERE), "csrc")

M3T_EINVAL = 10001
M3T_ESPIN = 10002
M3T_SCAN_NO_PERSIST = 1
M3T_BF16 = 2
M3T_GEMM_BESIDE_SCAN = 512
M3T_GEMM_F16X3 = 1024
M3T_GEMM_HIGH = 256
M3T_GEMM_EXCLUSIVE = 8
M3T_CONV_IMAGES = 4096
M3T_SCAN_FP32 = 4
M3T_SCAN_WHH = 8
M3T_SCAN_FAULT = 16
M3T_SCAN_WIDE = 32
M3T_MAX_SCANS = 8
M3T_JPEG_TRUNC, M3T_JPEG_CODE, M3T_JPEG_RST, M3T_JPEG_EXTRA = 1, 2, 4, 8

_f = C.c_void_p
_i = C.c_int
# ... 43 lines not shown
    "m3t_sgemm_bimg": [_i, _i, _i, _f, _i, _f, _f, _i, _f, _i, _i, _f, _z, _f, _f, _s],
    "m3t_sgemm_ring": [_i, _i, _i, _i, _i, _f, _i, _f, _i, _f, _i, _f, _i, _i, _i, _i, _i, _i, _f, _z, _i, _f, _f, _i, _s],
    "m3t_conv3d_taps_pre": [_f, _f, _f] + [_i] * 16 + [_f, _f, _f, _z, _f, _s],
    "m3t_conv3d_fwd_taps": [_f, _f, _f, _f] + [_i] * 15 + [_f, _f, _f, _z, _f, _s],
    "m3t_conv3d_fwd_taps4": [_f, _f, _f, _f] + [_i] * 14 + [_f, _f, _f, _z, _f, _s],
    "m3t_planes_to_cl4": [_f, _f, _i, _i, C.c_longlong, _s],
    "m3t_conv3d_wgrad_taps": [_f, _f, _f] + [_i] * 16 + [_f, _f, _f, _z, _s],
    "m3t_amax_out": [C.c_void_p],
    "m3t_colsum": [_f, _i, _i, _i, _f, _i, _f, _z, _s],
    "m3t_transpose": [_f, _i, _i, _i, _f, _i, _s],
    "m3t_relu_bwd": [_f, _f, _z, _s],
    "m3t_gru_scan_fwd": [C.POINTER(GruFwdDesc), _i, _i, _i, _f, _z, _i, _s],
    "m3t_gru_scan_bwd": [C.POINTER(GruBwdDesc), _i, _i, _i, _f, _z, _i, _s],
    "m3t_gru_bwd_prepare_floats": [_i],
    "m3t_gru_bwd_prepare": [C.POINTER(C.c_void_p), _i, _i, _i, C.POINTER(C.c_void_p), _s],
    "m3t_gru_persist_count": [],
    "m3t_gru_scan_workgroups": [_i, _i, _i, _i, _i, _i],
    "m3t_gru_poll_error": [],
    "m3t_gru_error_reset": [],
    "m3t_gru_error_defer": [_i],
    "m3t_gru_inject_error": [_s],
    "m3t_gru_persist_owner": [],
    "m3t_gru_scan_arena": [C.c_void_p, _z],
    "m3t_gru_scan_arena_reset": [C.c_void_p],
    "m3t_gru_scan_after": [C.c_void_p],
    "m3t_gru_scan_progress": [C.c_void_p, _i, C.POINTER(C.c_int), C.POINTER(C.c_uint)],
    "m3t_gru_scan_progress_reset": [C.c_void_p],
    "m3t_gru_scan_progress_ok": [_i, _i, _i, _i, _i, _i],
    "m3t_stream_wait_progress": [C.c_void_p, C.c_uint, _s],
    "m3t_gru_scan_events": [C.c_void_p, C.c_void_p],
    "m3t_gru_persist_profile": [C.c_void_p],
    "m3t_att_fuse_fwd": [_f, _f, _f, _f, _f, _i, _i, _s],
    "m3t_att_fuse_bwd": [_f, _f, _f, _f, _f, _f, _f, _f, _f, _i, _i, _s],
    "m3t_bn_cl_ws_bytes": [_z, _i],
    "m3t_bn_cl_fwd": [_f, _z, _i, _f, _f, _f, _f, C.c_float, C.c_float, _i, _i, _f, _f, _f, _f, _z, _s],
    "m3t_bn_cl_bwd": [_f, _f, _f, _f, _f, _f, _z, _i, _i, _i, _f, _f, _f, _f, _f, _z, _s],
    "m3t_bn_pool_cl_fwd": [_f, _z, _i, _i, _i, _i, _f, _f, _f, _f, C.c_float, C.c_float, _i, _f, C.c_void_p, _f, _f, _f, _z, _s],
    "m3t_bn_pool_cl_bwd": [_f, _f, _f, C.c_void_p, _f, _f, _f, _z, _i, _i, _i, _i, _i, _f, _f, _f, _f, _f, _z, _s],
    "m3t_pool_cl_fwd": [_f, _z, _i, _i, _i, _i, _i, _i, _i, _i, _i, _f, C.c_void_p, _s],
    "m3t_pool_cl_bwd": [_f, C.c_void_p, _z, _i, _i, _i, _i, _i, _i, _i, _i, _i, _f, _s],
    "m3t_bn_add_relu_cl_fwd": [_f, _f, _z, _i, _f, _f, _f, _f, C.c_float, C.c_float, _i, _f, _f, _f, _f, _z, _s],
    "m3t_bn_add_relu_cl_bwd": [_f, _f, _f, _f, _f, _f, _z, _i, _i, _f, _f, _f, _f, _f, _f, _z, _s],
    "m3t_mean_cl_fwd": [_f, _z, _i, _i, _f, _s],
    "m3t_mean_cl_bwd": [_f, _z, _i, _i, _f, _s],
    "m3t_gn_cl_ws_bytes": [_i, _z, _i],
    "m3t_gn_cl_fwd": [_f, _i, _z, _i, _i, _f, _f, C.c_float, _i, _f, _f, _f, _f, _z, _s],
    "m3t_gn_cl_bwd": [_f, _f, _f, _f, _f, _f, _i, _z, _i, _i, _i, _f, _f, _f, _f, _f, _z, _s],
    "m3t_gn_pool_cl_fwd": [_f, _i, _i, _i, _i, _i, _i, _i, _f, _f, C.c_float, _f, C.c_void_p, _f, _f, _f, _z, _s],
    "m3t_gn_pool_cl_bwd": [_f, _f, _f, C.c_void_p, _f, _f, _f, _i, _i, _i, _i, _i, _i, _i, _f, _f, _f, _f, _f, _z, _s],
    "m3t_relu_cl_ws_bytes": [_z, _i],
    "m3t_relu_cl_fwd": [_f, _z, _i, _f, _s],
    "m3t_relu_cl_bwd": [_f, _f, _z, _i, _f, _f, _f, _z, _s],
    "m3t_relu_pool_cl_fwd": [_f, _z, _i, _i, _i, _i, _f, C.c_void_p, _s],
    "m3t_relu_pool_cl_bwd": [_f, _f, C.c_void_p, _z, _i, _i, _i, _i, _f, _f, _f, _z, _s],
    "m3t_va_loss": [_f, _i, _i, _i, _i, _f, _f, _f, _f, _i, C.c_float, C.c_float, C.c_float, _i, _f, _f, _f, _z, _s],
    "m3t_va_loss_ws_bytes": [_i],
    "m3t_weight_norm_fwd": [_f, _f, _f, _f, _i, _i, _i, _s],
    "m3t_weight_norm_bwd": [_f, _f, _f, _f, _f, _f, _i, _i, _i, _s],
    "m3t_causal_conv_fwd": [_f, _f, _f, _f, _f, _f, _f, _i, _i, _i, _i, _i, _i, _i, _i, _s],
    "m3t_causal_conv_wgrad": [_f, _f, _f, _i, _i, _i, _i, _i, _i, _f, _z, _s],
    "m3t_conv1d_fwd": [_f, _f, _f, _f, _f, _f, _f, _i, _i, _i, _i, _i, _i, _i, _i, _i, C.c_float, C.c_ulonglong, _i, _s],
    "m3t_conv1d_fwd_scaled": [_f, _f, _f, _f, _f, _f, _f, _i, _i, _i, _i, _i, _i, _i, _i, _i, C.c_float, C.c_ulonglong, _i, _f, _f, _s],
    "m3t_conv1d_wgrad": [_f, _f, _f, _i, _i, _i, _i, _i, _i, _i, _f, _z, _i, _s],
    "m3t_conv1d_wgrad_scaled": [_f, _f, _f, _i, _i, _i, _i, _i, _i, _i, _f, _z, _i, _f, _f, _s],
    "m3t_pool_planes_fwd": [_f, C.c_longlong, _i, _i, _i, _i, _i, _i, _i, _i, _f, C.c_void_p, _s],
    "m3t_pool_planes_bwd": [_f, C.c_void_p, C.c_longlong, _i, _i, _i, _i, _i, _i, _i, _i, _f, _s],
# ... 133 lines not shown
```

### m3f.pytorch_amd/m3t/ops.py

```python
import ctypes as C
import os
import sys

import torch

from . import _lib
from ._lib import GruFwdDesc, GruBwdDesc, M3T_MAX_SCANS, M3THipError

_WS = {}
_WS_MIN = 64 << 20

PROFILE = []

import weakref

_GRAD_SINKS = {}


def register_grad_sink(param, view, owner=None):
    _GRAD_SINKS[id(param)] = [weakref.ref(param), view, False, id(owner) if owner is not None else None]


def clear_grad_sinks(owner=None):
    if owner is None:
# ... 222 lines not shown
    return "main"


def workspace(device, nbytes=_WS_MIN, tag=None):
    key = (device.type, device.index, tag or _ws_tag(device))
    ws = _WS.get(key)
    if ws is None or ws.numel() * 4 < nbytes:
        ws = torch.empty(max(nbytes, _WS_MIN) // 4, dtype=torch.float32, device=device)
        _WS[key] = ws
    return ws


_PREC = [_lib.M3T_GEMM_F16X3]


class precision:

    def __init__(self, mode):
        if mode not in ("fp32", "x6", "high", "bf16"):
            raise ValueError("precision mode must be 'fp32', 'x6', 'high' or 'bf16'")
        self.flag = {"fp32": _lib.M3T_GEMM_F16X3, "x6": 0, "high": _lib.M3T_GEMM_HIGH, "bf16": _lib.M3T_BF16}[mode]

    def __enter__(self):
        self.prev = _PREC[0]
        _PREC[0] = self.flag
        return self

    def __exit__(self, *exc):
        _PREC[0] = self.prev
        return False


def sgemm(transA, transB, M, N, K, A, a_off, lda, B, b_off, ldb, Cm, c_off, ldc, bias=None, act=0,
          accumulate=False, seg=(0, 0, 0, 0), use_ws=True, prec=None, exclusive=False, amax=(None, None)):
    ws = workspace(Cm.device) if use_ws else None
    flags = (_PREC[0] if prec is None else prec) | (_lib.M3T_GEMM_EXCLUSIVE if exclusive else 0)
    if _FENCED[0]:
        flags |= _lib.M3T_GEMM_BESIDE_SCAN
    with _Timed("sgemm_kernel", 1, 2.0 * M * N * K) if PROFILE_GEMM[0] else _NULL:
        rc = lib().m3t_sgemm_scaled(transA, transB, M, N, K, _p(A, a_off), lda, _p(B, b_off), ldb, _p(Cm, c_off), ldc,
                                    _p(bias), act, int(accumulate), seg[0], seg[1], seg[2], seg[3],
                                    _p(ws), (ws.numel() * 4) if ws is not None else 0, flags, amax[0], amax[1], _stream())
    _lib.check(rc, "m3t_sgemm")


_AMAX_ONE = {}


def amax_one(device):
    key = (device.type, device.index)
    t = _AMAX_ONE.get(key)
    if t is None:
        t = _AMAX_ONE[key] = torch.full((1,), 0x3F800000, dtype=torch.int64, device=device)
    return t.data_ptr()


_SLOT_POOL = {}
_SLOT_CHUNK = 8192


def amax_slots(n, device):
    key = (device.type, device.index)
    st = _SLOT_POOL.get(key)
    if st is None or st[1] + n > st[0].numel():
        st = _SLOT_POOL[key] = [torch.zeros(max(_SLOT_CHUNK, n), dtype=torch.int64, device=device), 0]
        if device.type == "cuda":
            ev = torch.cuda.Event()
            ev.record(cur_stream(device))
            others = ([_SIDE.get(key)] if _SIDE.get(key) is not None else []) + list(_WGRAD.get(key) or [])
            for other in others:
                other.wait_event(ev)
            st.append(ev)
            st.append({cur_stream(device).cuda_stream} | {o.cuda_stream for o in others})
    if len(st) > 3 and device.type == "cuda":
        h = _RAW_STREAM(device.index if device.index is not None else _CUR_DEV()) if _RAW_STREAM is not None else None
        if h is not None and h not in st[3]:
# ... 51 lines not shown

def _frozen_weight_amax(w, keep):
    if torch.is_grad_enabled() or not _W_AMAX_ON or not torch.is_tensor(w) or not w.is_cuda or w.dtype != torch.float32 or w.dim() < 2:
        return None
    e = _W_AMAX_FROZEN.get(id(w))
    if e is not None and e[0]() is w and e[2] == w._version and e[3] == w.data_ptr() and e[4] == _W_GEN[0]:
        slot = e[1]
    else:
        if not w.is_contiguous() or (w.numel() // w.shape[0]) % 4 != 0 or w.data_ptr() % 16 != 0:
            return None
        if len(_W_AMAX_FROZEN) > 4096:
            _W_AMAX_FROZEN.clear()
        slot = torch.zeros(1, dtype=torch.int64, device=w.device)
        if not measure_amax([(w.detach().view(w.shape[0], -1), slot.data_ptr())]):
            return None
        _W_AMAX_FROZEN[id(w)] = (weakref.ref(w), slot, w._version, w.data_ptr(), _W_GEN[0])
    if keep is not None and not any(k is slot for k in keep):
        keep.append(slot)
    return slot.data_ptr()


def _is_unit(x):
    v = getattr(x, "_m3t_unit", None)
    return v is not None and v is not False and v == x._version + 1


def _tagged_amax(x):
    e = getattr(x, "_m3t_amax", None)
    if e is None:
        return None
    return e[0] if e[1] == x._version else None


def measure_amax(items):
    for t, _ in items:
        if t.shape[-1] % 4 != 0 or t.data_ptr() % 16 != 0 or not t.is_contiguous():
            return False
    for i in range(0, len(items), 16):
        chunk = items[i:i + 16]
        n = len(chunk)
        xs = (C.c_void_p * n)(*[t.data_ptr() for t, _ in chunk])
        rows = (C.c_size_t * n)(*[t.numel() // t.shape[-1] for t, _ in chunk])
        cols = (C.c_int * n)(*[t.shape[-1] for t, _ in chunk])
        lds = (C.c_size_t * n)(*[t.shape[-1] for t, _ in chunk])
        sl = (C.c_void_p * n)(*[a for _, a in chunk])
        _lib.check(lib().m3t_absmax(n, xs, rows, cols, lds, sl, _stream()), "m3t_absmax")
    return True


def sgemm_plan(transA, M, N, K, seg_len=0, exclusive=False, prec=None, ws_bytes=_WS_MIN):
    k, sp = C.c_int(0), C.c_int(0)
    flags = (_PREC[0] if prec is None else prec) | (_lib.M3T_GEMM_EXCLUSIVE if exclusive else 0)
    _lib.check(lib().m3t_sgemm_plan(transA, M, N, K, seg_len, ws_bytes, flags, C.byref(k), C.byref(sp)), "m3t_sgemm_plan")
    return k.value, sp.value


def colsum(X, x_off, M, N, ld, out, accumulate=False):
    ws = workspace(out.device)
    rc = lib().m3t_colsum(_p(X, x_off), M, N, ld, _p(out), int(accumulate), _p(ws), ws.numel() * 4, _stream())
    _lib.check(rc, "m3t_colsum")


def transpose2d(src):
    R, Cc = src.shape
    dst = torch.empty(Cc, R, dtype=src.dtype, device=src.device)
    _lib.check(lib().m3t_transpose(_p(src), R, Cc, Cc, _p(dst), R, _stream()), "m3t_transpose")
# ... 1 lines not shown


def amax_out(slot):
    if slot is not None:
        _lib.check(lib().m3t_amax_out(C.c_void_p(slot)), "m3t_amax_out")


def _amax_clear():
    _lib.check(lib().m3t_amax_out(None), "m3t_amax_out")


def _armed_call(slot_ptr, entry, *args):
    amax_out(slot_ptr)
    try:
        _lib.check(getattr(lib(), entry)(*args), entry)
    except BaseException:
        _amax_clear()
        raise


def mask_pos(s, dy, mul=None, drop=None, amax=None):
    out = torch.empty_like(dy)
    if drop is not None and drop[0] > 0:
        Cc = dy.shape[-1]
        _armed_call(amax, "m3t_mask_pos_drop", _p(s), _p(dy), _p(out), dy.numel() // Cc, Cc, float(drop[0]), int(drop[1]), _stream())
    else:
        _armed_call(amax, "m3t_mask_pos", _p(s), _p(dy), _p(mul), _p(out), dy.numel(), _stream())
    return out


class _Linear(torch.autograd.Function):

    @staticmethod
    def forward(ctx, x, w, b, act, unit=False):
        x = _req(x.contiguous(), "x"); _req(w, "weight")
        K = x.shape[-1]
        N = w.shape[0]
        M = x.numel() // K
        y = torch.empty(x.shape[:-1] + (N,), dtype=x.dtype, device=x.device)
        ctx.prec = _PREC[0]
        slots = None
        ctx.w_slot = None
        if (ctx.prec & _lib.M3T_GEMM_F16X3) and M % 128 == 0 and N % 64 == 0 and K % 32 == 0 and w.is_contiguous():
            slots = amax_slots(3, x.device)
            ctx.w_keep = []
            ctx.w_slot = weight_amax(w, ctx.w_keep)
            ctx.x_slot = amax_one(x.device) if unit else slots.data_ptr()
            todo = ([] if unit else [(x, slots.data_ptr())]) + ([] if ctx.w_slot is not None else [(w, slots.data_ptr() + 8)])
            if todo and not measure_amax(todo):
                slots = None
            elif ctx.w_slot is None:
                ctx.w_slot = slots.data_ptr() + 8
        sgemm(0, 1, M, N, K, x, 0, K, w, 0, K, y, 0, N, bias=b, act=act, prec=ctx.prec, exclusive=True,
              amax=(None, None) if slots is None else (ctx.x_slot, ctx.w_slot))
        ctx.save_for_backward(x, w, y if act else None, slots)
        ctx.act, ctx.has_bias = act, b is not None
        ctx.bias_ref = b if (b is not None and id(b) in _GRAD_SINKS) else None
        ctx.weight_ref = w if id(w) in _GRAD_SINKS else None
        return y

    @staticmethod
    def backward(ctx, dy):
        x, w, y, slots = ctx.saved_tensors
        dy = _req(dy.contiguous(), "dy")
        if ctx.act:
            dy = mask_pos(y, dy)
        K, N = x.shape[-1], w.shape[0]
        M = x.numel() // K
        dx = dw = db = None
        a_x = a_w = a_dy = None
        if slots is not None and measure_amax([(dy, slots.data_ptr() + 16)]):
            a_x, a_w, a_dy = ctx.x_slot, ctx.w_slot, slots.data_ptr() + 16
        if ctx.needs_input_grad[0]:
            dx = torch.empty_like(x)
            sgemm(0, 0, M, K, N, dy, 0, N, w, 0, K, dx, 0, K, prec=ctx.prec, exclusive=True, amax=(a_dy, a_w))
        w_sink = _take_sink(ctx.weight_ref) if (ctx.needs_input_grad[1] and ctx.weight_ref is not None) else None
        b_sink = _take_sink(ctx.bias_ref) if (ctx.has_bias and ctx.needs_input_grad[2] and ctx.bias_ref is not None) else None
        if (ctx.needs_input_grad[1] and ctx.weight_ref is not None and w_sink is None) or \
                (ctx.has_bias and ctx.needs_input_grad[2] and ctx.bias_ref is not None and b_sink is None):
            join_wgrad(x.device)
        wg = wgrad_stream(x.device, _LINEAR_RR[0]) if x.is_cuda else None
        off_chain = on_stream(wg) if wg is not None else None
        if off_chain is not None and (w_sink is not None or b_sink is not None):
            wg.wait_stream(cur_stream())
        if ctx.needs_input_grad[1]:
            if w_sink is not None and off_chain is not None:
                with off_chain:
                    sgemm(1, 0, N, K, M, dy, 0, N, x, 0, K, w_sink, 0, K, prec=ctx.prec, amax=(a_dy, a_x))
                    if slots is not None:
                        slots.record_stream(wg)
            else:
                dw = w_sink if w_sink is not None else torch.empty_like(w)
                sgemm(1, 0, N, K, M, dy, 0, N, x, 0, K, dw, 0, K, prec=ctx.prec, exclusive=True, amax=(a_dy, a_x))
                if w_sink is not None:
                    dw = None
        if ctx.has_bias and ctx.needs_input_grad[2]:
            if b_sink is not None and off_chain is not None:
                with off_chain:
                    colsum(dy, 0, M, N, N, b_sink)
            else:
                db = b_sink if b_sink is not None else torch.empty(N, dtype=x.dtype, device=x.device)
                colsum(dy, 0, M, N, N, db)
                if b_sink is not None:
                    db = None
        if off_chain is not None and (w_sink is not None or b_sink is not None):
            dy.record_stream(wg)
            x.record_stream(wg)
            _WGRAD_PENDING[(x.device.type, x.device.index)] = True
            _LINEAR_RR[0] += 1
        return dx, dw, db, None, None


_LINEAR_RR = [0]


_NBT_PENDING = [None, 0]


def count_batch(counter):
    if counter is None:
        return
    if _NBT_PENDING[0] is not None:
        _NBT_PENDING[0].append(counter)
    else:
        counter.add_(1)


class batch_counters:
    def __enter__(self):
        if _NBT_PENDING[1] == 0:
            _NBT_PENDING[0] = []
        _NBT_PENDING[1] += 1
        return self

    def __exit__(self, *exc):
        _NBT_PENDING[1] -= 1
        if _NBT_PENDING[1] == 0:
            pending, _NBT_PENDING[0] = _NBT_PENDING[0], None
            if pending:
                counts = {}
                for t in pending:
                    e = counts.setdefault((t.device, t.data_ptr()), [t, 0])
                    e[1] += 1
# ... 25 lines not shown


def add_relu(a, b):
    if (a.is_cuda and a.dtype == torch.float32 and b.dtype == torch.float32 and a.shape == b.shape and a.device == b.device
            and a.is_contiguous() and b.is_contiguous()):
        _OUT_SLOT[0] = None
        return _tag_out(_AddRelu.apply(a, b))
    return torch.relu(a + b)


class _ReluDropout(torch.autograd.Function):

    @staticmethod
    def forward(ctx, y, p, seed):
        y = _req(y.contiguous(), "y")
        ctx.save_for_backward(y)
        ctx.drop = (float(p), int(seed))
        return mask_pos(y, y, drop=ctx.drop)

    @staticmethod
    def backward(ctx, dy):
        (y,) = ctx.saved_tensors
        return mask_pos(y, _req(dy.contiguous(), "dy"), drop=ctx.drop), None, None


def relu_dropout(y, p, seed=None):
    if p <= 0:
        return y
    if seed is None:
        seed = int(torch.empty(1, dtype=torch.int64).random_().item())
    return _ReluDropout.apply(y, float(p), int(seed))


def linear(x, w, b=None, act=0):
    return _Linear.apply(x, w, b, act, _is_unit(x))


SCAN_PER_STEP = [False]
SCAN_FAULT = [False]
RANGE_PROBE = [[] if os.environ.get("M3T_F16X3_PROBE") == "1" else None]


def _probe_range(tag, t2d):
    a = t2d.abs()
    rmax, cmax, gmax = a.amax(1), a.amax(0), a.max()
    big = torch.full((), float("inf"), device=t2d.device)
    lim = gmax * 2.0 ** -17
    sq = t2d.double() ** 2
    tot = sq.sum()
    past_r, past_c = rmax < lim, cmax < lim
    RANGE_PROBE[0].append((tag, gmax, torch.where(rmax > 0, rmax, big).min(), torch.where(cmax > 0, cmax, big).min(),
                           past_r.sum(), past_c.sum(), sq.sum(1)[past_r].sum() / tot, sq.sum(0)[past_c].sum() / tot))


def range_probe_report(clear=True):
    keys = ("tag", "max", "row_spread", "col_spread", "rows_past", "cols_past", "row_energy_past", "col_energy_past")
    out = []
    for rec in (RANGE_PROBE[0] or []):
        v = [rec[0]] + [float(x) for x in rec[1:]]
        v[2], v[3] = v[1] / v[2], v[1] / v[3]
        out.append(dict(zip(keys, v)))
    if clear and RANGE_PROBE[0] is not None:
        RANGE_PROBE[0] = []
    return out


PREP_AHEAD = [os.environ.get("M3T_SCAN_PREP_AHEAD", "1") != "0"]
SCAN_FIRST = [os.environ.get("M3T_SCAN_FIRST", "0") == "1"]
# ... 255 lines not shown

class _MultiBiGRU(torch.autograd.Function):

    @staticmethod
    def forward(ctx, n_stacks, L, cat_lo, cat_hi, unit_mask, *tensors):
        per = 1 + 8 * L
        assert len(tensors) == n_stacks * per
        xs, params = [], []
        for s in range(n_stacks):
            xs.append(_req(tensors[s * per].contiguous(), "x"))
            params.append([_req(t, "gru parameter") for t in tensors[s * per + 1:(s + 1) * per]])
        B, T = xs[0].shape[0], xs[0].shape[1]
        dev = xs[0].device
        for x in xs:
            if x.shape[0] != B or x.shape[1] != T:
                raise M3THipError("grouped GRU stacks must share batch and length")
        Hs = [params[s][1].shape[1] for s in range(n_stacks)]
        new = lambda *shape: torch.empty(*shape, dtype=torch.float32, device=dev)
        h_ns = [new(2 * L, B, Hs[s]) for s in range(n_stacks)]
        outs = [[new(B, T, 2 * Hs[s]) for s in range(n_stacks)] for _ in range(L)]
        cat_buf = None
        if cat_hi - cat_lo >= 2:
            cat_buf = new(B, T, sum(2 * Hs[s] for s in range(cat_lo, cat_hi)))
            off = 0
            for s in range(cat_lo, cat_hi):
                outs[L - 1][s] = cat_buf[..., off:off + 2 * Hs[s]]
                off += 2 * Hs[s]
        gates = [[new(2, B, T, 4 * Hs[s]) for s in range(n_stacks)] for _ in range(L)]
        xprojs = [[new(B, T, 6 * Hs[s]) for s in range(n_stacks)] for _ in range(L)]
        main = cur_stream()
        prec = _PREC[0]
        groups = _stream_groups(Hs, B)
        fslots = None
        if (prec & _lib.M3T_GEMM_F16X3) and all(h % 4 == 0 for h in Hs):
            fslots = amax_slots(n_stacks * (1 + 2 * L), dev)
            items = [(xs[s], fslots.data_ptr() + 8 * s) for s in range(n_stacks) if not (unit_mask >> s) & 1]
            wslot = {}
            ctx.w_keep = []
            for l in range(L):
                for s in range(n_stacks):
                    for d in (0, 1):
                        a = weight_amax(params[s][(2 * l + d) * 4], ctx.w_keep)
                        if a is None:
                            a = fslots.data_ptr() + 8 * (n_stacks + (l * n_stacks + s) * 2 + d)
                            items.append((params[s][(2 * l + d) * 4], a))
                        wslot[(l, s, d)] = a
            if not measure_amax(items):
                fslots = None
        one = amax_one(dev)

        def fslot_x(l, s):
            return None if fslots is None else (fslots.data_ptr() + 8 * s if (l == 0 and not (unit_mask >> s) & 1) else one)

        def fslot_w(l, s, d):
            return None if fslots is None else wslot[(l, s, d)]

        alone = not _interleaved(groups) and all(kind == "main" for kind, _ in groups)

        def level_fwd(l, idxs, scan, after=None, wide=False, progress=None):
            descs = []
            for s in idxs:
                H = Hs[s]
                inp = xs[s] if l == 0 else outs[l - 1][s]
                I = inp.shape[-1]
                for d in (0, 1):
                    w_ih, w_hh, b_ih, b_hh = params[s][(2 * l + d) * 4:(2 * l + d) * 4 + 4]
                    if not scan:
                        sgemm(0, 1, B * T, 3 * H, I, inp, 0, I, w_ih, 0, I, xprojs[l][s], d * 3 * H, 6 * H, bias=b_ih, prec=prec,
                              exclusive=alone, amax=(fslot_x(l, s), fslot_w(l, s, d)))
                    else:
                        descs.append(GruFwdDesc(_vp(xprojs[l][s]), _vp(w_hh), _vp(b_hh), _vp(outs[l][s]),
                                                _vp(gates[l][s], d * B * T * 4 * H), _vp(h_ns[s], (2 * l + d) * B * H),
                                                H, d, 6 * H, d * 3 * H, outs[l][s].stride(1), d * H))
            if scan:
                return _scan_fwd(descs, B, T, prec | (_lib.M3T_SCAN_WIDE if (wide or FORCE_WIDE_FWD[0]) else 0), after,
                                 None if progress is None else (_progress_counters(dev), progress))

        def chunk_plan(idxs, wide):
            if L < 2 or fslots is None or len({Hs[i] for i in idxs}) != 1 or 2 * len(idxs) > M3T_MAX_SCANS:
                return None
            H = Hs[idxs[0]]
            if H % 64 != 0:
                return None
            fl = _scan_flags(dev) | prec | (_lib.M3T_SCAN_WIDE if (wide or FORCE_WIDE_FWD[0]) else 0)
# ... 184 lines not shown
            out, gts = acts[(l * n_stacks + s) * 2], acts[(l * n_stacks + s) * 2 + 1]
            inp = xs[s] if l == 0 else acts[((l - 1) * n_stacks + s) * 2]
            return inp, out, gts

        dev = params[0][0].device
        new = lambda *shape: torch.empty(*shape, dtype=torch.float32, device=dev)
        out_grads = [None] * (n_stacks * per)
        sunk = [False] * (n_stacks * per)
        douts, dhns = [], []
        cat_lo, cat_hi = ctx.cat
        dcat = None
        if cat_hi > cat_lo:
            g = grads[2 * cat_lo]
            dcat = (torch.zeros(B, T, sum(2 * Hs[s] for s in range(cat_lo, cat_hi)), dtype=torch.float32, device=dev) if g is None
                    else _req(g.contiguous(), "dout"))
        off = 0
        for s in range(n_stacks):
            g, gh = grads[2 * s], grads[2 * s + 1]
            if dcat is not None and cat_lo <= s < cat_hi:
                douts.append(dcat[..., off:off + 2 * Hs[s]])
                off += 2 * Hs[s]
            else:
                douts.append(torch.zeros(B, T, 2 * Hs[s], dtype=torch.float32, device=dev) if g is None
                             else _req(g.contiguous(), "dout"))
            dhns.append(None if gh is None else _req(gh.contiguous(), "dh_n"))
        dgx = [[new(B, T, 6 * Hs[s]) for s in range(n_stacks)] for _ in range(L)]
        dgh = [[new(2, B, T, 3 * Hs[s]) for s in range(n_stacks)] for _ in range(L)]
        dh = [[new(2, B, Hs[s]) for s in range(n_stacks)] for _ in range(L)]
        dbp = [[new(2, B, 4, Hs[s]) for s in range(n_stacks)] for _ in range(L)]
        direct_whh = all(h % 16 == 0 for h in Hs) and all(p.is_contiguous() for prm in params for p in prm)
        wht = [[[None if direct_whh else new(Hs[s], 3 * Hs[s]) for _ in (0, 1)] for s in range(n_stacks)] for _ in range(L)]
        need_dx = [[l > 0 or ctx.needs_input_grad[5 + s * per] for s in range(n_stacks)] for l in range(L)]
        dinp = [[torch.empty_like(layer_io(l, s)[0]) if need_dx[l][s] else None for s in range(n_stacks)] for l in range(L)]
        for s in range(n_stacks):
            for l in range(L):
                for d in (0, 1):
                    w_ih, w_hh = params[s][(2 * l + d) * 4], params[s][(2 * l + d) * 4 + 1]
                    base = s * per + 1 + (2 * l + d) * 4
                    for j, prm in enumerate(params[s][(2 * l + d) * 4:(2 * l + d) * 4 + 4]):
                        sink = _take_sink(prm)
                        out_grads[base + j] = sink if sink is not None else torch.empty_like(prm)
                        sunk[base + j] = sink is not None
        main = cur_stream()
        groups = _stream_groups(Hs, B)
        cur = {s: douts[s] for s in range(n_stacks)}
        prec = ctx.prec
        wfq = ctx.wfq or {}
        if ctx.wfq_ev is not None:
            main.wait_event(ctx.wfq_ev)
        NSL = _CHUNK_WINDOWS + 1
        bslots = amax_slots(2 * L * n_stacks * NSL, dev) if fslots is not None else None
        one = amax_one(dev)

        def bslot(l, s, d, j=-1):
            return None if bslots is None else bslots.data_ptr() + 8 * (((l * n_stacks + s) * 2 + d) * NSL + 1 + j)

        def fslot_x(l, s):
            return None if fslots is None else (fslots.data_ptr() + 8 * s if (l == 0 and not (ctx.unit_mask >> s) & 1) else one)

        def fslot_w(l, s, d):
            return None if fslots is None else ctx.wslot[(l, s, d)]

        def chunk_plan(l, idxs):
            if bslots is None or len({Hs[i] for i in idxs}) != 1 or 2 * len(idxs) > M3T_MAX_SCANS or not any(need_dx[l][s] for s in idxs):
                return None
            H = Hs[idxs[0]]
            if H % 64 != 0 or any(need_dx[l][s] and layer_io(l, s)[0].shape[-1] % 64 != 0 for s in idxs) or not direct_whh:
                return None
            fl = _scan_flags(dev) | prec | _lib.M3T_SCAN_WHH | _lib.M3T_SCAN_WIDE
            if not lib().m3t_gru_scan_progress_ok(2 * len(idxs), H, B, T, fl, 1):
                return None
            tb = _chunk_bounds(B, T, backward=True)
            return tb if (tb is not None and len(tb) + 1 <= _CHUNK_WINDOWS) else None

        def dx_pieces(l, idxs, tb, need, scan_stream):
            wg = wgs[1]
            ctr = _progress_counters(dev)
            ev_end = torch.cuda.Event()
            ev_end.record(scan_stream)
            lo, hi = [0] + tb, tb + [T]
            n = len(tb)
            with on_stream(wg):
                ended = False
                for dirn, k, w, second in _arrivals(tb, T):
                    if k is None:
                        if not ended:
                            wg.wait_event(ev_end)
                            ended = True
                    else:
                        _wait_progress(ctr, dirn, need[dirn * n + k])
                    d = 1 - dirn
                    j = w if dirn == 0 else n - w
                    by_shape = {}
                    for si in idxs:
                        if need_dx[l][si]:
                            I = layer_io(l, si)[0].shape[-1]
# ... 45 lines not shown
                                            _vp(w_hh if direct_whh else wht[l][s][d]),
                                            _vp(dhns[s], (2 * l + d) * B * H) if dhns[s] is not None else None,
                                            _vp(dgx[l][s]), _vp(dgh[l][s], d * B * T * 3 * H), _vp(dh[l][s], d * B * H),
                                            _vp(dbp[l][s], d * B * 4 * H), _vp(out_grads[base + 2]), _vp(out_grads[base + 3]),
                                            H, d, out.stride(1), d * H, 6 * H, d * 3 * H, bslot(l, s, d),
                                            _vp(wfq[(l, s, d)]) if (l, s, d) in wfq else None))
            chain = _ws_tag(dev)
            sm = None
            if progress is None and chain in held:
                sm = start_marks(idxs)
            need = _scan_bwd(descs, B, T, prec | (_lib.M3T_SCAN_WHH if direct_whh else 0) | _lib.M3T_SCAN_WIDE, after,
                             None if (progress is None and sm is None) else (_progress_counters(dev), progress if progress is not None else sm))
            if progress is not None:
                pending[(l, tuple(idxs))] = (progress, need)
            release_held(chain, (_progress_counters(dev), need) if sm is not None else None)
            if RANGE_PROBE[0] is not None:
                for s in idxs:
                    for d in (0, 1):
                        _probe_range("dgx l%d s%d d%d H%d" % (l, s, d, Hs[s]), dgx[l][s].view(B * T, 6 * Hs[s])[:, d * 3 * Hs[s]:(d + 1) * 3 * Hs[s]])
                        _probe_range("dgh l%d s%d d%d H%d" % (l, s, d, Hs[s]), dgh[l][s][d].view(B * T, 3 * Hs[s]))

        pending = {}

        def level_dx(l, idxs):
            pg = pending.pop((l, tuple(idxs)), None)
            if pg is not None:
                dx_pieces(l, idxs, pg[0], pg[1], cur_stream())
                return
            for s in idxs:
                H = Hs[s]
                inp, out, gts = layer_io(l, s)
                I = inp.shape[-1]
                if need_dx[l][s]:
                    for d in (0, 1):
                        sgemm(0, 0, B * T, I, 3 * H, dgx[l][s], d * 3 * H, 6 * H, params[s][(2 * l + d) * 4], 0, I,
                              dinp[l][s], 0, I, accumulate=(d == 1), prec=prec, amax=(bslot(l, s, d), fslot_w(l, s, d)))
                    cur[s] = dinp[l][s]

        wgs = wgrad_streams(dev)
        rr = [0]

        def _level_dw(l, idxs, pool):
            for s in idxs:
                H = Hs[s]
                inp, out, gts = layer_io(l, s)
                I = inp.shape[-1]
                for d in (0, 1):
                    base = s * per + 1 + (2 * l + d) * 4
                    dw_ih, dw_hh = out_grads[base:base + 2]
                    goff = d * B * T * 3 * H
                    with (on_stream(pool[rr[0] % len(pool)]) if pool is not None else _NULL):
                        if T > 1:
                            a_off, b_off = (1, 0) if d == 0 else (0, 1)
                            sgemm(1, 0, 3 * H, H, B * (T - 1), dgh[l][s], goff, 3 * H, out, d * H, out.stride(1), dw_hh, 0, H,
                                  seg=(T - 1, T, a_off, b_off), prec=prec, amax=(bslot(l, s, d), one if bslots is not None else None))
                        else:
                            dw_hh.zero_()
                    rr[0] += 1
                    with (on_stream(pool[rr[0] % len(pool)]) if pool is not None else _NULL):
                        sgemm(1, 0, 3 * H, I, B * T, dgx[l][s], d * 3 * H, 6 * H, inp, 0, I, dw_ih, 0, I, prec=prec,
                              amax=(bslot(l, s, d), fslot_x(l, s)))
                    rr[0] += 1

        def level_dw(l, idxs, spread=False, wg_i=0):
            if spread:
                _level_dw(l, idxs, [cur_stream(), wgs[1]])
            else:
                with on_stream(wgs[wg_i]):
                    _level_dw(l, idxs, None)
# ... 65 lines not shown
                    ev_heavy = torch.cuda.Event()
                    ev_heavy.record(main)
                    level_gemms(l, heavy)
                    with on_stream(side):
                        level_scan(l, light, ev_heavy)
                        ev_light = torch.cuda.Event()
                        ev_light.record(side)
                        level_gemms(l, light)
            finally:
                _FENCED[0] = False
            main.wait_stream(side)
        else:
            for kind, idxs in groups:
                stream = main
                if kind == "side":
                    stream = side_stream(dev)
                    stream.wait_stream(main)
                with on_stream(stream):
                    for l in range(L - 1, -1, -1):
                        level_scan(l, idxs, progress=chunk_plan(l, idxs) if (kind == "main" and len(groups) == 1) else None)
                        level_gemms(l, idxs)
            for kind, _ in groups:
                if kind == "side":
                    main.wait_stream(side_stream(dev))
        for key_ in list(held):
            release_held(key_, None)
        weights_sunk = all(sunk[s * per + 1 + (2 * l + d) * 4 + j] for s in range(n_stacks) for l in range(L) for d in (0, 1) for j in (0, 1))
        if weights_sunk:
            for l in range(L):
                for s in range(n_stacks):
                    for t in (dgx[l][s], dgh[l][s]) + tuple(layer_io(l, s)[:2]):
                        for w_ in wgs:
                            t.record_stream(w_)
            for t in (bslots, fslots):
                if t is not None:
                    for w_ in wgs:
                        t.record_stream(w_)
            _WGRAD_PENDING[(dev.type, dev.index)] = True
        else:
            for w_ in wgs:
                main.wait_stream(w_)
        for s in range(n_stacks):
            out_grads[s * per] = dinp[0][s]
        return (None, None, None, None, None) + tuple(None if sunk[i] else g for i, g in enumerate(out_grads))


def multi_bigru(stacks, cat=None):
    L = stacks[0][2]
    flat = []
    for x, prm, l in stacks:
        if l != L:
            raise M3THipError("grouped GRU stacks must have the same depth")
        flat.append(x)
        flat.extend(prm)
    lo, hi = cat if cat is not None else (0, 0)
    unit_mask = sum(1 << i for i, (x, _, _) in enumerate(stacks) if _is_unit(x))
    res = _MultiBiGRU.apply(len(stacks), L, lo, hi, unit_mask, *flat)
    for i in range(len(stacks)):
        if res[2 * i].numel():
            res[2 * i]._m3t_unit = res[2 * i]._version + 1
    return [(res[2 * i], res[2 * i + 1]) for i in range(len(stacks))]


class _AttFuse(torch.autograd.Function):

    @staticmethod
    def forward(ctx, s_v, s_a, x_v, x_a):
        s_v, s_a = _req(s_v.contiguous(), "s_v"), _req(s_a.contiguous(), "s_a")
        x_v, x_a = _req(x_v.contiguous(), "x_v"), _req(x_a.contiguous(), "x_a")
        D = x_v.shape[-1]
        rows = x_v.numel() // D
        if x_a.shape != x_v.shape or s_v.numel() != rows or s_a.numel() != rows:
            raise M3THipError("att_fuse: shape mismatch")
        f = torch.empty_like(x_v)
        with _Timed("att_fuse_fwd_kernel", 1, 0, nbytes=4.0 * rows * (3 * D + 2)):
            _lib.check(lib().m3t_att_fuse_fwd(_p(s_v), _p(s_a), _p(x_v), _p(x_a), _p(f), rows, D, _stream()), "m3t_att_fuse_fwd")
        ctx.save_for_backward(s_v, s_a, x_v, x_a)
        return f

    @staticmethod
    def backward(ctx, df):
        s_v, s_a, x_v, x_a = ctx.saved_tensors
        df = _req(df.contiguous(), "df")
        D = x_v.shape[-1]
        rows = x_v.numel() // D
        ds_v, ds_a = torch.empty_like(s_v), torch.empty_like(s_a)
        dx_v, dx_a = torch.empty_like(x_v), torch.empty_like(x_a)
        with _Timed("att_fuse_bwd_kernel", 1, 0, nbytes=4.0 * rows * (5 * D + 4)):
            _lib.check(lib().m3t_att_fuse_bwd(_p(df), _p(s_v), _p(s_a), _p(x_v), _p(x_a), _p(ds_v), _p(ds_a), _p(dx_v),
                                              _p(dx_a), rows, D, _stream()), "m3t_att_fuse_bwd")
        return ds_v, ds_a, dx_v, dx_a


def att_fuse(s_v, s_a, x_v, x_a):
    return _AttFuse.apply(s_v, s_a, x_v, x_a)


class _VALoss(torch.autograd.Function):
    @staticmethod
    def forward(ctx, y_hat, valence, arousal, class_expr, expr_valid, iv, ia, n_expr, w_v, w_a, expr_w, use_mse):
        y = _req(y_hat.contiguous(), "y_hat")
        Cc = y.shape[-1]
        rows = y.numel() // Cc
        val = _req(valence.contiguous().float(), "valence")
        aro = _req(arousal.contiguous().float(), "arousal")
        cls = vld = None
        if n_expr > 0:
            cls = class_expr.contiguous().long()
            vld = expr_valid.contiguous().to(torch.uint8)
            if not cls.is_cuda or not vld.is_cuda:
                raise M3THipError("labels must be device tensors")
        stats = torch.empty(8, dtype=torch.float32, device=y.device)
        dy = torch.empty_like(y)
        ws = workspace(y.device)
        with _Timed("va_loss_kernels", 3, 0, nbytes=4.0 * rows * (3 * Cc + 3 * 2 + Cc) + (3.0 * rows * 9 if n_expr > 0 else 0.0)):
            rc = lib().m3t_va_loss(_p(y), rows, Cc, iv, ia, _p(val), _p(aro),
                                   C.c_void_p(cls.data_ptr()) if cls is not None else None,
                                   C.c_void_p(vld.data_ptr()) if vld is not None else None,
                                   n_expr, w_v, w_a, expr_w, int(use_mse), _p(stats), _p(dy), _p(ws), ws.numel() * 4, _stream())
        _lib.check(rc, "m3t_va_loss")
        ctx.save_for_backward(dy)
        ctx.mark_non_differentiable(stats)
        return stats[0], stats

    @staticmethod
    def backward(ctx, g_loss, g_stats):
        (dy,) = ctx.saved_tensors
        return (dy * g_loss,) + (None,) * 11
# ... 2180 lines not shown
```

### m3f.pytorch_amd/m3t/workloads.py

```python
import os

import torch
import torch.nn as nn

from . import ops
from models.rnn import GRU, run_grus, run_grus_cat
from models.att_fusion import AttFusion
from models.tcn import TemporalConvNet


class AVFeatureGraph(nn.Module):

    def __init__(self, d_a=128, d_v=256, num_hidden=512, fc_outputs=9, num_fc_layers=2):
        super().__init__()
        self.audio = GRU(d_a, 256, 2, -1, num_fc_layers)
        self.visual = nn.Module()
        self.visual.gru_v = GRU(d_v, num_hidden, 2, -1, num_fc_layers)
        self.visual.gru_a = GRU(d_v, num_hidden, 2, -1, num_fc_layers)
        self.proj_v = nn.Linear(num_hidden * 4, 512)
        self.att_fuse = AttFusion([512, 512], 128)
        self.fusion = GRU(512, num_hidden, 2, fc_outputs, num_fc_layers)

    def forward(self, x_a, x_v):
        a, v12 = run_grus_cat([self.audio, self.visual.gru_v, self.visual.gru_a], [x_a, x_v, x_v], 1, 3)
        v = ops.linear(v12, self.proj_v.weight, self.proj_v.bias, 0)
        return self.fusion(self.att_fuse(a, v))


class TcnHead(nn.Module):

    def __init__(self, d_in=128, hidden=512, levels=2):
        super().__init__()
        self.tcn = nn.ModuleList([TemporalConvNet(d_in, [hidden] * levels, 3), nn.Linear(hidden, 2)])

    def forward(self, x):
        h = self.tcn[0].forward_btc(ops.bct_to_btc(x))
        return ops.linear(h, self.tcn[1].weight, self.tcn[1].bias, 0)


class TcnGru(nn.Module):

    def __init__(self, d_in=256, hidden=512):
        super().__init__()
        self.tcn = TemporalConvNet(d_in, [hidden, hidden], 3)
        self.gru = GRU(hidden, hidden, 2, 2, 2)

    def forward(self, x):
        return self.gru(self.tcn.forward_btc(ops.bct_to_btc(x)))


def c3_bucket_order(model):
    return [list(model.fusion.parameters()),
            list(model.att_fuse.parameters()) + list(model.proj_v.parameters()),
            list(model.visual.parameters()) + list(model.audio.parameters())]


def make_c3_step(model, batch, max_norm=1.0, **ddp_kw):
    from .ddp import FlatGradDDP
# ... 36 lines not shown
```

### m3f.pytorch_amd/models/att_fusion.py

```python
import torch.nn as nn

from m3t import ops
from .rnn import GRU, run_grus


class AttFusion(nn.Module):
    def __init__(self, input_dim=[512, 512], hidden_dim=128):
        super().__init__()
        d_audio, d_video = input_dim[0], input_dim[1]
        self.use_proj = d_video != d_audio
        if self.use_proj:
            self.proj_v = nn.Linear(d_video, d_audio)
        self.scorer_a = GRU(d_audio, hidden_dim, 1, 1, 1)
        self.scorer_v = GRU(d_audio, hidden_dim, 1, 1, 1)

    def forward(self, x_a, x_v):
        if self.use_proj:
            x_v = ops.linear(x_v, self.proj_v.weight, self.proj_v.bias, 0)
        s_v, s_a = run_grus([self.scorer_v, self.scorer_a], [x_v, x_a])
        return ops.att_fuse(s_v, s_a, x_v, x_a)
```

Measured before the change: 2847.

## Fuse attention scorer heads into att_fuse kernel and share dx accumulation

Adds fused forward and backward kernels that compute the Linear(2H,1) scorer heads directly inside the attention-fusion kernel, so the separate head GEMMs and kernel launches go away. The fused kernels also fold the output amax tracking needed by fp16x3 scaling into the pass, along with the split-k reduce and GEMM paths, which removes separate absmax passes. The backward pass writes the scorer GRU input gradients into shared buffers via accumulate instead of adding them separately. The cost is more complex autograd plumbing through global side-channel state and accumulate-into semantics that can go wrong.

```diff
diff --git a/include/m3t_hip.h b/include/m3t_hip.h
--- a/include/m3t_hip.h
+++ b/include/m3t_hip.h
@@ -161,6 +161,11 @@
                      const float* x_v, const float* x_a,
                      float* ds_v, float* ds_a, float* dx_v, float* dx_a,
                      int rows, int D, void* stream);
+int m3t_att_fuse_scored_fwd(const float* o_v, const float* o_a, const float* w_v, const float* w_a, const float* b_v, const float* b_a,
+                            const float* x_v, const float* x_a, float* f, float* s_v, float* s_a, int rows, int D, int S, void* stream);
+int m3t_att_fuse_scored_bwd(const float* df, const float* s_v, const float* s_a, const float* x_v, const float* x_a,
+                            const float* w_v, const float* w_a, float* ds_v, float* ds_a, float* dx_v, float* dx_a,
+                            float* do_v, float* do_a, int rows, int D, int S, void* stream);
 
 int m3t_va_loss(const float* y_hat, int rows, int C, int iv, int ia,
                 const float* valence, const float* arousal,
diff --git a/m3f.pytorch_amd/csrc/fuse_loss.hip b/m3f.pytorch_amd/csrc/fuse_loss.hip
--- a/m3f.pytorch_amd/csrc/fuse_loss.hip
+++ b/m3f.pytorch_amd/csrc/fuse_loss.hip
@@ -79,6 +79,111 @@
         const float dot = w0 * d0 + w1 * d1;
         ds_v[row] = w0 * (d0 - dot) * hv * (1.f - hv);
         ds_a[row] = w1 * (d1 - dot) * ha * (1.f - ha);
+    }
+}
+
+__device__ __forceinline__ float head_score(const float* __restrict__ o, const float* __restrict__ w, const float* __restrict__ b, int S, int lane) {
+    float acc = 0.f;
+    for (int i = lane; i < S; i += 64) acc = fmaf(o[i], w[i], acc);
+    return wave_sum(acc) + (b ? b[0] : 0.f);
+}
+
+__global__ __launch_bounds__(256) void att_fuse_scored_fwd_kernel(const float* __restrict__ o_v, const float* __restrict__ o_a,
+                                                                  const float* __restrict__ w_v, const float* __restrict__ w_a,
+                                                                  const float* __restrict__ b_v, const float* __restrict__ b_a,
+                                                                  const float* __restrict__ x_v, const float* __restrict__ x_a,
+                                                                  float* __restrict__ f, float* __restrict__ s_v, float* __restrict__ s_a,
+                                                                  int rows, int D, int S, int vec, unsigned long long* amax) {
+    const int lane = threadIdx.x & 63;
+    const int row = blockIdx.x * 4 + (threadIdx.x >> 6);
+    float mx = 0.f;
+    if (row < rows) {
+        const float sv = head_score(o_v + (size_t)row * S, w_v, b_v, S, lane);
+        const float sa = head_score(o_a + (size_t)row * S, w_a, b_a, S, lane);
+        if (lane == 0) { s_v[row] = sv; s_a[row] = sa; }
+        float hv, ha, w0, w1;
+        fuse_weights(sv, sa, hv, ha, w0, w1);
+        const size_t base = (size_t)row * D;
+        if (vec) {
+            const float4* pv = reinterpret_cast<const float4*>(x_v + base);
+            const float4* pa = reinterpret_cast<const float4*>(x_a + base);
+            float4* pf = reinterpret_cast<float4*>(f + base);
+            for (int i = lane; i < (D >> 2); i += 64) {
+                const float4 v = pv[i], a = pa[i];
+                const float4 o = make_float4(mix2(w0, v.x, w1, a.x), mix2(w0, v.y, w1, a.y), mix2(w0, v.z, w1, a.z), mix2(w0, v.w, w1, a.w));
+                pf[i] = o;
+                mx = fmaxf(fmaxf(mx, m3t_fin_abs(o.x)), fmaxf(m3t_fin_abs(o.y), fmaxf(m3t_fin_abs(o.z), m3t_fin_abs(o.w))));
+            }
+        } else {
+            for (int i = lane; i < D; i += 64) {
+                const float o = mix2(w0, x_v[base + i], w1, x_a[base + i]);
+                f[base + i] = o;
+                mx = fmaxf(mx, m3t_fin_abs(o));
+            }
+        }
+    }
+    __shared__ float red4[4];
+    if (amax) m3t_block_raise_slot(amax, mx, red4);
+}
+
+__global__ __launch_bounds__(256) void att_fuse_scored_bwd_kernel(const float* __restrict__ df, const float* __restrict__ s_v,
+                                                                  const float* __restrict__ s_a, const float* __restrict__ x_v,
+                                                                  const float* __restrict__ x_a, const float* __restrict__ w_v,
+                                                                  const float* __restrict__ w_a, float* __restrict__ ds_v,
+                                                                  float* __restrict__ ds_a, float* __restrict__ dx_v, float* __restrict__ dx_a,
+                                                                  float* __restrict__ do_v, float* __restrict__ do_a, int rows, int D, int S,
+                                                                  int vec, int vec_s) {
+    const int lane = threadIdx.x & 63;
+    const int row = blockIdx.x * 4 + (threadIdx.x >> 6);
+    if (row >= rows) return;
+    float hv, ha, w0, w1;
+    fuse_weights(s_v[row], s_a[row], hv, ha, w0, w1);
+    const size_t base = (size_t)row * D;
+    float d0 = 0.f, d1 = 0.f;
+    if (vec) {
+        const float4* pg = reinterpret_cast<const float4*>(df + base);
+        const float4* pv = reinterpret_cast<const float4*>(x_v + base);
+        const float4* pa = reinterpret_cast<const float4*>(x_a + base);
+        float4* qv = reinterpret_cast<float4*>(dx_v + base);
+        float4* qa = reinterpret_cast<float4*>(dx_a + base);
+        for (int i = lane; i < (D >> 2); i += 64) {
+            const float4 g = pg[i], v = pv[i], a = pa[i];
+            d0 += g.x * v.x + g.y * v.y + g.z * v.z + g.w * v.w;
+            d1 += g.x * a.x + g.y * a.y + g.z * a.z + g.w * a.w;
+            qv[i] = make_float4(w0 * g.x, w0 * g.y, w0 * g.z, w0 * g.w);
+            qa[i] = make_float4(w1 * g.x, w1 * g.y, w1 * g.z, w1 * g.w);
+        }
+    } else {
+        for (int i = lane; i < D; i += 64) {
+            const float g = df[base + i];
+            d0 += g * x_v[base + i];
+            d1 += g * x_a[base + i];
+            dx_v[base + i] = w0 * g;
+            dx_a[base + i] = w1 * g;
+        }
+    }
+    d0 = wave_sum(d0);
+    d1 = wave_sum(d1);
+    const float dot = w0 * d0 + w1 * d1;
+    const float gv = w0 * (d0 - dot) * hv * (1.f - hv);
+    const float ga = w1 * (d1 - dot) * ha * (1.f - ha);
+    if (lane == 0) { ds_v[row] = gv; ds_a[row] = ga; }
+    const size_t sb = (size_t)row * S;
+    if (vec_s) {
+        const float4* pwv = reinterpret_cast<const float4*>(w_v);
+        const float4* pwa = reinterpret_cast<const float4*>(w_a);
+        float4* qv = reinterpret_cast<float4*>(do_v + sb);
+        float4* qa = reinterpret_cast<float4*>(do_a + sb);
+        for (int i = lane; i < (S >> 2); i += 64) {
+            const float4 a = pwv[i], b = pwa[i];
+            qv[i] = make_float4(gv * a.x, gv * a.y, gv * a.z, gv * a.w);
+            qa[i] = make_float4(ga * b.x, ga * b.y, ga * b.z, ga * b.w);
+        }
+    } else {
+        for (int i = lane; i < S; i += 64) {
+            do_v[sb + i] = gv * w_v[i];
+            do_a[sb + i] = ga * w_a[i];
+        }
     }
 }
 
@@ -532,6 +637,33 @@
     return 0;
 }
 
+extern "C" int m3t_att_fuse_scored_fwd(const float* o_v, const float* o_a, const float* w_v, const float* w_a, const float* b_v,
+                                       const float* b_a, const float* x_v, const float* x_a, float* f, float* s_v, float* s_a, int rows,
+                                       int D, int S, void* stream) {
+    unsigned long long* amax = m3t_take_amax_out();
+    if (rows <= 0 || D <= 0) return 0;
+    if (S <= 0 || !o_v || !o_a || !w_v || !w_a || !x_v || !x_a || !f || !s_v || !s_a || (uintptr_t)amax % 8 != 0) return M3T_EINVAL;
+    const int vec = (D % 4 == 0) && (((uintptr_t)x_v | (uintptr_t)x_a | (uintptr_t)f) % 16 == 0);
+    att_fuse_scored_fwd_kernel<<<cdiv(rows, 4), 256, 0, (hipStream_t)stream>>>(o_v, o_a, w_v, w_a, b_v, b_a, x_v, x_a, f, s_v, s_a, rows, D,
+                                                                                S, vec, amax);
+    M3T_LAUNCH_CHECK();
+    return 0;
+}
+
+extern "C" int m3t_att_fuse_scored_bwd(const float* df, const float* s_v, const float* s_a, const float* x_v, const float* x_a,
+                                       const float* w_v, const float* w_a, float* ds_v, float* ds_a, float* dx_v, float* dx_a,
+                                       float* do_v, float* do_a, int rows, int D, int S, void* stream) {
+    if (rows <= 0 || D <= 0) return 0;
+    if (S <= 0 || !df || !s_v || !s_a || !x_v || !x_a || !w_v || !w_a || !ds_v || !ds_a || !dx_v || !dx_a || !do_v || !do_a) return M3T_EINVAL;
+    const int vec = (D % 4 == 0) &&
+                    (((uintptr_t)x_v | (uintptr_t)x_a | (uintptr_t)df | (uintptr_t)dx_v | (uintptr_t)dx_a) % 16 == 0);
+    const int vec_s = (S % 4 == 0) && (((uintptr_t)w_v | (uintptr_t)w_a | (uintptr_t)do_v | (uintptr_t)do_a) % 16 == 0);
+    att_fuse_scored_bwd_kernel<<<cdiv(rows, 4), 256, 0, (hipStream_t)stream>>>(df, s_v, s_a, x_v, x_a, w_v, w_a, ds_v, ds_a, dx_v, dx_a,
+                                                                                do_v, do_a, rows, D, S, vec, vec_s);
+    M3T_LAUNCH_CHECK();
+    return 0;
+}
+
 extern "C" size_t m3t_va_loss_ws_bytes(int rows) { return rows > 0 ? (size_t)cdiv(rows, LB) * 16 * sizeof(double) : 0; }
 
 extern "C" int m3t_va_loss(const float* y_hat, int rows, int C, int iv, int ia, const float* valence,
diff --git a/m3f.pytorch_amd/csrc/gemm.hip b/m3f.pytorch_amd/csrc/gemm.hip
--- a/m3f.pytorch_amd/csrc/gemm.hip
+++ b/m3f.pytorch_amd/csrc/gemm.hip
@@ -235,8 +235,9 @@
 }
 
 __global__ void splitk_reduce_kernel(const float* __restrict__ ws, float* __restrict__ C, const float* __restrict__ bias,
-                                     int M, int N, int ldc, int splits, int act, int accumulate) {
+                                     int M, int N, int ldc, int splits, int act, int accumulate, unsigned long long* amax) {
     const size_t total = (size_t)M * N;
+    float mx = 0.f;
     for (size_t i = blockIdx.x * (size_t)blockDim.x + threadIdx.x; i < total; i += (size_t)gridDim.x * blockDim.x) {
         const int m = (int)(i / N), n = (int)(i % N);
         float s = 0.f;
@@ -246,7 +247,10 @@
         float* q = C + (size_t)m * ldc + n;
         if (accumulate) s += *q;
         *q = s;
-    }
+        if (amax) mx = fmaxf(mx, m3t_fin_abs(s));
+    }
+    __shared__ float red4[4];
+    if (amax) m3t_block_raise_slot(amax, mx, red4);
 }
 
 constexpr int SK_FOLD = 32;
@@ -273,10 +277,11 @@
 
 __global__ __launch_bounds__(256) void splitk_reduce4_kernel(const float* __restrict__ ws, float* __restrict__ C,
                                                              const float* __restrict__ bias, int M, int N, int ldc, int splits,
-                                                             int act, int accumulate, int kstride) {
+                                                             int act, int accumulate, int kstride, unsigned long long* amax) {
     const size_t total4 = (size_t)M * N / 4, slab4 = total4 * (size_t)kstride;
     const float4* w4 = reinterpret_cast<const float4*>(ws);
     const int n4 = N / 4;
+    float mx = 0.f;
     for (size_t i = blockIdx.x * (size_t)blockDim.x + threadIdx.x; i < total4; i += (size_t)gridDim.x * blockDim.x) {
         float4 s = make_float4(0.f, 0.f, 0.f, 0.f);
         int k = 0;
@@ -297,7 +302,10 @@
         float4* q = reinterpret_cast<float4*>(C + (size_t)m * ldc + n);
         if (accumulate) { const float4 c = *q; s.x += c.x; s.y += c.y; s.z += c.z; s.w += c.w; }
         *q = s;
-    }
+        if (amax) mx = fmaxf(fmaxf(mx, m3t_fin_abs(s.x)), fmaxf(m3t_fin_abs(s.y), fmaxf(m3t_fin_abs(s.z), m3t_fin_abs(s.w))));
+    }
+    __shared__ float red4[4];
+    if (amax) m3t_block_raise_slot(amax, mx, red4);
 }
 
 
@@ -356,7 +364,7 @@
 }
 
 static void launch_splitk_reduce(const float* ws, float* C, const float* bias, int M, int N, int ldc, int splits, int act,
-                                 int accumulate, hipStream_t s) {
+                                 int accumulate, hipStream_t s, unsigned long long* amax = nullptr) {
     const size_t total = (size_t)M * N;
     if (N % 4 == 0 && ldc % 4 == 0 && ((uintptr_t)C % 16) == 0 && ((uintptr_t)ws % 16) == 0) {
         int blocks = (int)((total / 4 + 255) / 256);
@@ -364,15 +372,15 @@
         if (splits >= 4 * SK_FOLD && blocks <= 64) {
             const int groups = (splits + SK_FOLD - 1) / SK_FOLD;
             splitk_fold4_kernel<<<dim3(blocks, groups), 256, 0, s>>>(const_cast<float*>(ws), total / 4, splits);
-            splitk_reduce4_kernel<<<blocks, 256, 0, s>>>(ws, C, bias, M, N, ldc, groups, act, accumulate, SK_FOLD);
+            splitk_reduce4_kernel<<<blocks, 256, 0, s>>>(ws, C, bias, M, N, ldc, groups, act, accumulate, SK_FOLD, amax);
             return;
         }
-        splitk_reduce4_kernel<<<blocks, 256, 0, s>>>(ws, C, bias, M, N, ldc, splits, act, accumulate, 1);
+        splitk_reduce4_kernel<<<blocks, 256, 0, s>>>(ws, C, bias, M, N, ldc, splits, act, accumulate, 1, amax);
         return;
     }
     int blocks = (int)((total + 255) / 256);
     if (blocks > 2048) blocks = 2048;
-    splitk_reduce_kernel<<<blocks, 256, 0, s>>>(ws, C, bias, M, N, ldc, splits, act, accumulate);
+    splitk_reduce_kernel<<<blocks, 256, 0, s>>>(ws, C, bias, M, N, ldc, splits, act, accumulate, amax);
 }
 
 __global__ void colsum_kernel(const float* __restrict__ X, int M, int N, int ld, float* __restrict__ out, int accumulate) {
@@ -546,17 +554,17 @@
 int m3t_sgemm_x6_launch(int transA, int transB, int M, int N, int K, const float* A, int lda, const float* B, int ldb,
                         float* C, int ldc, const float* bias, int act, int accumulate, int seg_len, int seg_stride,
                         int a_off, int b_off, float* ws, int splits, int kchunk, size_t dyn_lds, int bf16_operands, int narrow,
-                        const unsigned long long* amax_a, const unsigned long long* amax_b, hipStream_t s);
+                        const unsigned long long* amax_a, const unsigned long long* amax_b, hipStream_t s, unsigned long long* amax_c);
 
 int m3t_sgemm_x6d_launch(int transA, int transB, int M, int N, int K, const float* A, int lda, const float* B, int ldb,
                          float* C, int ldc, const float* bias, int act, int accumulate, int seg_len, int seg_stride,
                          int a_off, int b_off, float* ws, int splits, int kchunk, int bf16_operands,
-                         const unsigned long long* amax_a, const unsigned long long* amax_b, hipStream_t s);
+                         const unsigned long long* amax_a, const unsigned long long* amax_b, hipStream_t s, unsigned long long* amax_c);
 
 int m3t_sgemm_x6w_launch(int transA, int transB, int M, int N, int K, const float* A, int lda, const float* B, int ldb,
                          float* C, int ldc, const float* bias, int act, int accumulate, int seg_len, int seg_stride,
                          int a_off, int b_off, float* ws, int splits, int kchunk, int bf16_operands,
-                         const unsigned long long* amax_a, const unsigned long long* amax_b, hipStream_t s);
+                         const unsigned long long* amax_a, const unsigned long long* amax_b, hipStream_t s, unsigned long long* amax_c);
 
 static int x6d_mode() { return 2; }
 
@@ -655,6 +663,12 @@
     return 0;
 }
 
+static bool amax_after_ok(const float* C, int N, int ldc) { return N % 4 == 0 && ldc % 4 == 0 && (uintptr_t)C % 16 == 0; }
+static int amax_after(unsigned long long* slot, const float* C, int M, int N, int ldc, hipStream_t s) {
+    const M3TRegion r{C, (unsigned long long)M, (unsigned long long)ldc, N / 4, slot};
+    return m3t_absmax_regions(&r, 1, s);
+}
+
 extern "C" int m3t_sgemm(int transA, int transB, int M, int N, int K, const float* A, int lda, const float* B, int ldb,
                          float* C, int ldc, const float* bias, int act, int accumulate, int seg_len, int seg_stride,
                          int a_off, int b_off, float* ws, size_t ws_bytes, int flags, void* stream) {
@@ -666,9 +680,11 @@
                                 float* C, int ldc, const float* bias, int act, int accumulate, int seg_len, int seg_stride,
                                 int a_off, int b_off, float* ws, size_t ws_bytes, int flags, const unsigned long long* amax_a,
                                 const unsigned long long* amax_b, void* stream) {
+    unsigned long long* amax_c = m3t_take_amax_out();
     if (M <= 0 || N <= 0) return 0;
     if (K < 0 || !A || !B || !C) return M3T_EINVAL;
     if (seg_len > 0 && !(transA == 1 && transB == 0)) return M3T_EINVAL;
+    if (amax_c && (uintptr_t)amax_c % 8 != 0) return M3T_EINVAL;
     GemmParams p;
     p.A = A; p.B = B; p.C = C; p.bias = bias; p.ws = ws;
     p.M = M; p.N = N; p.K = K; p.lda = lda; p.ldb = ldb; p.ldc = ldc;
@@ -713,21 +729,22 @@
         }
         if (g.wide || wide_tr)
             rc = m3t_sgemm_x6w_launch(transA, transB, M, N, K, A, lda, B, ldb, C, ldc, bias, act, accumulate, seg_len, seg_stride,
-                                      a_off, b_off, ws, splits, kchunk, f16x3 ? 3 : 0, use_a, use_b, s);
+                                      a_off, b_off, ws, splits, kchunk, f16x3 ? 3 : 0, use_a, use_b, s, amax_c);
         else if (!g.narrow && K % 32 == 0 && (!f16x3 || f16x3_on_x6d()) && !(flags & (M3T_GEMM_BACKGROUND | M3T_GEMM_HIGH)) && (x6d_mode() == 1 || (x6d_mode() == 2 && !(flags & M3T_GEMM_BESIDE_SCAN))))
             rc = m3t_sgemm_x6d_launch(transA, transB, M, N, K, A, lda, B, ldb, C, ldc, bias, act, accumulate, seg_len, seg_stride,
-                                      a_off, b_off, ws, splits, kchunk, p.bf16 ? 1 : ((flags & M3T_GEMM_HIGH) ? 2 : (f16x3 ? 3 : 0)), use_a, use_b, s);
+                                      a_off, b_off, ws, splits, kchunk, p.bf16 ? 1 : ((flags & M3T_GEMM_HIGH) ? 2 : (f16x3 ? 3 : 0)), use_a, use_b, s, amax_c);
         else
             rc = m3t_sgemm_x6_launch(transA, transB, M, N, K, A, lda, B, ldb, C, ldc, bias, act, accumulate, seg_len, seg_stride,
                                      a_off, b_off, ws, splits, kchunk, (flags & M3T_GEMM_BACKGROUND) ? (size_t)40 * 1024 : 0,
-                                     p.bf16 ? 1 : ((flags & M3T_GEMM_HIGH) ? 2 : (f16x3 ? 3 : 0)), g.narrow, use_a, use_b, s);
+                                     p.bf16 ? 1 : ((flags & M3T_GEMM_HIGH) ? 2 : (f16x3 ? 3 : 0)), g.narrow, use_a, use_b, s, amax_c);
         if (rc) return rc;
         if (splits > 1) {
-            launch_splitk_reduce(ws, C, bias, M, N, ldc, splits, act, accumulate, s);
+            launch_splitk_reduce(ws, C, bias, M, N, ldc, splits, act, accumulate, s, amax_c);
             M3T_LAUNCH_CHECK();
         }
         return 0;
     }
+    if (amax_c && !amax_after_ok(C, N, ldc)) return M3T_EINVAL;
     dim3 grid(tn, tm, splits), block(256);
     const bool fast = (M % BM == 0) && (N % BN == 0) && (K % BK == 0) && K > 0 && p.vecA && p.vecB;
     const size_t dyn = (flags & M3T_GEMM_BACKGROUND) ? (size_t)56 * 1024 + 0 : 0;
@@ -745,9 +762,9 @@
 #undef M3T_GEMM_LAUNCH
     M3T_LAUNCH_CHECK();
     if (splits > 1) {
-        launch_splitk_reduce(ws, C, bias, M, N, ldc, splits, act, accumulate, s);
+        launch_splitk_reduce(ws, C, bias, M, N, ldc, splits, act, accumulate, s, amax_c);
         M3T_LAUNCH_CHECK();
-    }
+    } else if (amax_c) return amax_after(amax_c, C, M, N, ldc, s);
     return 0;
 }
 
@@ -756,6 +773,7 @@
 
 extern "C" int m3t_sgemm_window_batch(int n, const m3t_window_problem* pr, int transB, int n_seg, int win_len, int win_stride, int win_off,
                                       int N, int K, int lda, int ldb, int ldc, int act, int flags, void* stream) {
+    if (m3t_take_amax_out()) return M3T_EINVAL;
     if (n <= 0 || n_seg <= 0 || win_len <= 0 || N <= 0) return 0;
     if (n > M3T_WINDOW_BATCH || !pr || K <= 0 || win_stride < win_len || win_off < 0 || win_off + win_len > win_stride) return M3T_EINVAL;
     const long long Ml = (long long)n_seg * win_len;
@@ -867,12 +885,16 @@
 extern "C" int m3t_sgemm_pre(int M, int N, int K, const float* A_img, int lda, const float* B_img, int ldb, float* C, int ldc,
                              const float* bias, int act, int accumulate, const unsigned long long* amax_a, const unsigned long long* amax_b,
                              void* stream) {
+    unsigned long long* amax_c = m3t_take_amax_out();
     if (M <= 0 || N <= 0) return 0;
+    if (amax_c && ((uintptr_t)amax_c % 8 != 0 || !amax_after_ok(C, N, ldc))) return M3T_EINVAL;
     if (!A_img || !B_img || !C || !amax_a || !amax_b || K <= 0 || !x6_enabled() || !m3t_f16x3_enabled() || M % 128 != 0 || N % 64 != 0 ||
         K % 32 != 0 || lda % 4 != 0 || ldb % 4 != 0 || (uintptr_t)A_img % 16 != 0 || (uintptr_t)B_img % 16 != 0)
         return M3T_EINVAL;
     const int narrow = (N % 128 != 0 || (long long)(M / 128) * (N / 128) <= 384) ? 1 : 0;
-    return m3t_sgemm_x6_pre_launch(M, N, K, A_img, lda, B_img, ldb, C, ldc, bias, act, accumulate, narrow, amax_a, amax_b, (hipStream_t)stream);
+    const int rc = m3t_sgemm_x6_pre_launch(M, N, K, A_img, lda, B_img, ldb, C, ldc, bias, act, accumulate, narrow, amax_a, amax_b, (hipStream_t)stream);
+    if (rc || !amax_c) return rc;
+    return amax_after(amax_c, C, M, N, ldc, (hipStream_t)stream);
 }
 
 namespace {
@@ -920,7 +942,9 @@
 extern "C" int m3t_sgemm_bimg(int M, int N, int K, const float* A, int lda, const float* B_img, float* C, int ldc, const float* bias, int act,
                               int accumulate, float* ws, size_t ws_bytes, const unsigned long long* amax_a, const unsigned long long* amax_b,
                               void* stream) {
+    unsigned long long* amax_c = m3t_take_amax_out();
     if (M <= 0 || N <= 0) return 0;
+    if (amax_c && ((uintptr_t)amax_c % 8 != 0 || !C || !amax_after_ok(C, N, ldc))) return M3T_EINVAL;
     if (!A || !B_img || !C || !amax_b || K <= 0 || !x6_enabled() || !m3t_f16x3_enabled() || M % 128 != 0 || N % 256 != 0 || K % 32 != 0 ||
         lda % 4 != 0 || (uintptr_t)A % 16 != 0 || (uintptr_t)B_img % 16 != 0)
         return M3T_EINVAL;
@@ -936,7 +960,8 @@
     const int splits = g.wide ? g.splits : 1, kchunk = g.wide ? g.kchunk : K;
     const int rc = m3t_sgemm_x6w_bimg_launch(M, N, K, A, lda, B_img, C, ldc, bias, act, accumulate, ws, splits, kchunk, use_a, use_b, s);
     if (rc) return rc;
-    if (splits > 1) { launch_splitk_reduce(ws, C, bias, M, N, ldc, splits, act, accumulate, s); M3T_LAUNCH_CHECK(); }
+    if (splits > 1) { launch_splitk_reduce(ws, C, bias, M, N, ldc, splits, act, accumulate, s, amax_c); M3T_LAUNCH_CHECK(); }
+    else if (amax_c) return amax_after(amax_c, C, M, N, ldc, s);
     return 0;
 }
 
@@ -948,7 +973,9 @@
                               const float* bias, int act, int accumulate, int seg_len, int seg_stride, int a_off, int b_off, float* ws,
                               size_t ws_bytes, int splits, const unsigned long long* amax_a, const unsigned long long* amax_b, int variant,
                               void* stream) {
+    unsigned long long* amax_c = m3t_take_amax_out();
     if (M <= 0 || N <= 0) return 0;
+    if (amax_c && ((uintptr_t)amax_c % 8 != 0 || !C || !amax_after_ok(C, N, ldc))) return M3T_EINVAL;
     if (!A || !B || !C || K <= 0 || !m3t_f16x3_enabled() || N % 256 != 0 || K % 16 != 0 || lda % 4 != 0 || ldb % 4 != 0 ||
         (uintptr_t)A % 16 != 0 || (uintptr_t)B % 16 != 0 || splits < 1)
         return M3T_EINVAL;
@@ -972,7 +999,8 @@
     const int rc = m3t_sgemm_ring_launch(transA, transB, M, N, K, A, lda, B, ldb, C, ldc, bias, act, accumulate, seg_len, seg_stride, a_off, b_off,
                                          ws, splits, kchunk, use_a, use_b, variant, s);
     if (rc) return rc;
-    if (splits > 1) { launch_splitk_reduce(ws, C, bias, M, N, ldc, splits, act, accumulate, s); M3T_LAUNCH_CHECK(); }
+    if (splits > 1) { launch_splitk_reduce(ws, C, bias, M, N, ldc, splits, act, accumulate, s, amax_c); M3T_LAUNCH_CHECK(); }
+    else if (amax_c) return amax_after(amax_c, C, M, N, ldc, s);
     return 0;
 }
 
diff --git a/m3f.pytorch_amd/csrc/gemm_x6.hip b/m3f.pytorch_amd/csrc/gemm_x6.hip
--- a/m3f.pytorch_amd/csrc/gemm_x6.hip
+++ b/m3f.pytorch_amd/csrc/gemm_x6.hip
@@ -507,7 +507,20 @@
                 *q = v;
             }
         }
-    if (CONV && p.cv_amax) {
+    if ((CONV || direct) && p.cv_amax) {
+        if (!CONV) {
+            asm volatile("s_waitcnt vmcnt(0)" ::: "memory");
+#pragma unroll
+            for (int i = 0; i < 2; ++i)
+#pragma unroll
+                for (int j = 0; j < NJ; ++j)
+#pragma unroll
+                    for (int r = 0; r < 16; ++r) {
+                        const int row = bm + wm * 64 + i * 32 + (r & 3) + 8 * (r >> 2) + 4 * hi;
+                        if (C3ROWS && row >= p.M) continue;
+                        vmax = fmaxf(vmax, m3t_fin_abs(dst[(size_t)(MW ? rowmap[row - bm] : row) * ldd + bn + wn * 32 * NJ + j * 32 + l31]));
+                    }
+        }
         __shared__ float red4[4];
         m3t_block_raise_slot(p.cv_amax, vmax, red4);
     }
@@ -520,7 +533,7 @@
 int m3t_sgemm_x6_launch(int transA, int transB, int M, int N, int K, const float* A, int lda, const float* B, int ldb,
                         float* C, int ldc, const float* bias, int act, int accumulate, int seg_len, int seg_stride,
                         int a_off, int b_off, float* ws, int splits, int kchunk, size_t dyn_lds, int bf16_operands, int narrow,
-                        const unsigned long long* amax_a, const unsigned long long* amax_b, hipStream_t s) {
+                        const unsigned long long* amax_a, const unsigned long long* amax_b, hipStream_t s, unsigned long long* amax_c) {
     X6Params p;
     p.amax_a = amax_a; p.amax_b = amax_b;
     p.A = A; p.B = B; p.C = C; p.bias = bias; p.ws = ws;
@@ -529,7 +542,7 @@
     p.seg_len = seg_len; p.seg_stride = seg_stride; p.a_off = a_off; p.b_off = b_off;
     p.cv_T = p.cv_C = p.cv_K = p.cv_dil = p.cv_lead = p.cv_anti = 0; p.cv_btap = 0; p.cv_mask = p.cv_res = nullptr; p.cv_pre = nullptr;
     p.cv_drop = m3t_make_drop(0.f, 0ull);
-    p.cv_amax = nullptr;
+    p.cv_amax = splits == 1 ? amax_c : nullptr;
     p.mw_len = p.mw_stride = p.mw_off = 0;
     p.c3_T = p.c3_H = p.c3_W = p.c3_To = p.c3_Ho = p.c3_Wo = p.c3_kt = p.c3_kh = p.c3_kw = p.c3_bt = p.c3_bh = p.c3_bw = p.c3_sg = p.c3_C = 0; p.c3_st = p.c3_sh = p.c3_sw = 1; p.tr_S = 0;
     dim3 grid(N / (narrow ? 64 : XN), M / XM, splits), block(256);
diff --git a/m3f.pytorch_amd/csrc/gemm_x6d.hip b/m3f.pytorch_amd/csrc/gemm_x6d.hip
--- a/m3f.pytorch_amd/csrc/gemm_x6d.hip
+++ b/m3f.pytorch_amd/csrc/gemm_x6d.hip
@@ -34,6 +34,7 @@
     M3TDrop cv_drop;
     const unsigned long long* amax_a;
     const unsigned long long* amax_b;
+    unsigned long long* amax_c;
 };
 
 typedef _Float16 f16x2 __attribute__((ext_vector_type(2)));
@@ -329,6 +330,21 @@
                 *q = v;
             }
         }
+    if (!CONV && direct && p.amax_c) {
+        asm volatile("s_waitcnt vmcnt(0) lgkmcnt(0)" ::: "memory");
+        float vmax = 0.f;
+#pragma unroll
+        for (int i = 0; i < 2; ++i)
+#pragma unroll
+            for (int j = 0; j < 2; ++j)
+#pragma unroll
+                for (int r = 0; r < 16; ++r) {
+                    const int row = bm + wm * 64 + i * 32 + (r & 3) + 8 * (r >> 2) + 4 * hi;
+                    vmax = fmaxf(vmax, m3t_fin_abs(dst[(size_t)row * ldd + bn + wn * 64 + j * 32 + l31]));
+                }
+        __syncthreads();
+        m3t_block_raise_slot(p.amax_c, vmax, reinterpret_cast<float*>(ldsb));
+    }
 }
 
 }
@@ -336,9 +352,10 @@
 int m3t_sgemm_x6d_launch(int transA, int transB, int M, int N, int K, const float* A, int lda, const float* B, int ldb,
                          float* C, int ldc, const float* bias, int act, int accumulate, int seg_len, int seg_stride,
                          int a_off, int b_off, float* ws, int splits, int kchunk, int bf16_operands,
-                         const unsigned long long* amax_a, const unsigned long long* amax_b, hipStream_t s) {
+                         const unsigned long long* amax_a, const unsigned long long* amax_b, hipStream_t s, unsigned long long* amax_c) {
     X6DParams p;
     p.amax_a = amax_a; p.amax_b = amax_b;
+    p.amax_c = splits == 1 ? amax_c : nullptr;
     if (bf16_operands == 3 && (!amax_a || !amax_b)) return M3T_EINVAL;
     p.A = A; p.B = B; p.C = C; p.bias = bias; p.ws = ws;
     p.M = M; p.N = N; p.K = K; p.lda = lda; p.ldb = ldb; p.ldc = ldc;
@@ -382,7 +399,7 @@
                         float* pre, int B, int T, int Ci, int Co, int K, int dil, int lead, int act, int anti, int bf16_operands,
                         M3TDrop drop, hipStream_t s) {
     X6DParams p;
-    p.amax_a = p.amax_b = nullptr;
+    p.amax_a = p.amax_b = nullptr; p.amax_c = nullptr;
     p.A = x; p.B = w_t; p.C = y; p.bias = bias; p.ws = nullptr;
     p.M = B * T; p.N = Co; p.K = K * Ci; p.lda = Ci; p.ldb = anti ? Co : Ci; p.ldc = Co;
     p.act = act; p.accumulate = 0; p.splits = 1; p.kchunk = K * Ci;
diff --git a/m3f.pytorch_amd/csrc/gemm_x6w.hip b/m3f.pytorch_amd/csrc/gemm_x6w.hip
--- a/m3f.pytorch_amd/csrc/gemm_x6w.hip
+++ b/m3f.pytorch_amd/csrc/gemm_x6w.hip
@@ -33,6 +33,7 @@
     int seg_len, seg_stride, a_off, b_off;
     const unsigned long long* amax_a;
     const unsigned long long* amax_b;
+    unsigned long long* amax_c;
 };
 
 template <int NS>
@@ -345,6 +346,21 @@
                 *q = v;
             }
         }
+    if (direct && p.amax_c) {
+        asm volatile("s_waitcnt vmcnt(0) lgkmcnt(0)" ::: "memory");
+        float vmax = 0.f;
+#pragma unroll
+        for (int i = 0; i < 2; ++i)
+#pragma unroll
+            for (int j = 0; j < 4; ++j)
+#pragma unroll
+                for (int r = 0; r < 16; ++r) {
+                    const int row = bm + wm * 64 + i * 32 + (r & 3) + 8 * (r >> 2) + 4 * hi;
+                    vmax = fmaxf(vmax, m3t_fin_abs(dst[(size_t)row * ldd + bn + wn * 128 + j * 32 + l31]));
+                }
+        __syncthreads();
+        m3t_block_raise_slot(p.amax_c, vmax, reinterpret_cast<float*>(ldsb));
+    }
 }
 
 }
@@ -352,11 +368,12 @@
 int m3t_sgemm_x6w_launch(int transA, int transB, int M, int N, int K, const float* A, int lda, const float* B, int ldb,
                          float* C, int ldc, const float* bias, int act, int accumulate, int seg_len, int seg_stride,
                          int a_off, int b_off, float* ws, int splits, int kchunk, int bf16_operands,
-                         const unsigned long long* amax_a, const unsigned long long* amax_b, hipStream_t s) {
+                         const unsigned long long* amax_a, const unsigned long long* amax_b, hipStream_t s, unsigned long long* amax_c) {
     if (bf16_operands != 0 && bf16_operands != 3) return M3T_EINVAL;
     if (bf16_operands == 3 && (!amax_a || !amax_b)) return M3T_EINVAL;
     X6WParams p;
     p.amax_a = amax_a; p.amax_b = amax_b;
+    p.amax_c = splits == 1 ? amax_c : nullptr;
     p.A = A; p.B = B; p.C = C; p.bias = bias; p.ws = ws;
     p.M = M; p.N = N; p.K = K; p.lda = lda; p.ldb = ldb; p.ldc = ldc;
     p.act = act; p.accumulate = accumulate; p.splits = splits; p.kchunk = kchunk;
@@ -397,7 +414,7 @@
                               const unsigned long long* amax_b, hipStream_t s) {
     if (!amax_a || !amax_b) return M3T_EINVAL;
     X6WParams p;
-    p.amax_a = amax_a; p.amax_b = amax_b;
+    p.amax_a = amax_a; p.amax_b = amax_b; p.amax_c = nullptr;
     p.A = A; p.B = B_img; p.C = C; p.bias = bias; p.ws = ws;
     p.M = M; p.N = N; p.K = K; p.lda = lda; p.ldb = 0; p.ldc = ldc;
     p.act = act; p.accumulate = accumulate; p.splits = splits; p.kchunk = kchunk;
diff --git a/m3f.pytorch_amd/m3t/_lib.py b/m3f.pytorch_amd/m3t/_lib.py
--- a/m3f.pytorch_amd/m3t/_lib.py
+++ b/m3f.pytorch_amd/m3t/_lib.py
@@ -99,6 +99,8 @@
     "m3t_gru_persist_profile": [C.c_void_p],
     "m3t_att_fuse_fwd": [_f, _f, _f, _f, _f, _i, _i, _s],
     "m3t_att_fuse_bwd": [_f, _f, _f, _f, _f, _f, _f, _f, _f, _i, _i, _s],
+    "m3t_att_fuse_scored_fwd": [_f] * 11 + [_i, _i, _i, _s],
+    "m3t_att_fuse_scored_bwd": [_f] * 13 + [_i, _i, _i, _s],
     "m3t_bn_cl_ws_bytes": [_z, _i],
     "m3t_bn_cl_fwd": [_f, _z, _i, _f, _f, _f, _f, C.c_float, C.c_float, _i, _i, _f, _f, _f, _f, _z, _s],
     "m3t_bn_cl_bwd": [_f, _f, _f, _f, _f, _f, _z, _i, _i, _i, _f, _f, _f, _f, _f, _z, _s],
diff --git a/m3f.pytorch_amd/m3t/ops.py b/m3f.pytorch_amd/m3t/ops.py
--- a/m3f.pytorch_amd/m3t/ops.py
+++ b/m3f.pytorch_amd/m3t/ops.py
@@ -278,16 +278,15 @@
 
 
 def sgemm(transA, transB, M, N, K, A, a_off, lda, B, b_off, ldb, Cm, c_off, ldc, bias=None, act=0,
-          accumulate=False, seg=(0, 0, 0, 0), use_ws=True, prec=None, exclusive=False, amax=(None, None)):
+          accumulate=False, seg=(0, 0, 0, 0), use_ws=True, prec=None, exclusive=False, amax=(None, None), amax_c=None):
     ws = workspace(Cm.device) if use_ws else None
     flags = (_PREC[0] if prec is None else prec) | (_lib.M3T_GEMM_EXCLUSIVE if exclusive else 0)
     if _FENCED[0]:
         flags |= _lib.M3T_GEMM_BESIDE_SCAN
     with _Timed("sgemm_kernel", 1, 2.0 * M * N * K) if PROFILE_GEMM[0] else _NULL:
-        rc = lib().m3t_sgemm_scaled(transA, transB, M, N, K, _p(A, a_off), lda, _p(B, b_off), ldb, _p(Cm, c_off), ldc,
-                                    _p(bias), act, int(accumulate), seg[0], seg[1], seg[2], seg[3],
-                                    _p(ws), (ws.numel() * 4) if ws is not None else 0, flags, amax[0], amax[1], _stream())
-    _lib.check(rc, "m3t_sgemm")
+        _armed_call(amax_c, "m3t_sgemm_scaled", transA, transB, M, N, K, _p(A, a_off), lda, _p(B, b_off), ldb, _p(Cm, c_off), ldc,
+                    _p(bias), act, int(accumulate), seg[0], seg[1], seg[2], seg[3],
+                    _p(ws), (ws.numel() * 4) if ws is not None else 0, flags, amax[0], amax[1], _stream())
 
 
 _AMAX_ONE = {}
@@ -405,6 +404,11 @@
     return e[0] if e[1] == x._version else None
 
 
+def _tagged_slot(x):
+    e = _tagged_amax(x) if (torch.is_tensor(x) and x.is_contiguous()) else None
+    return e if torch.is_tensor(e) else None
+
+
 def measure_amax(items):
     for t, _ in items:
         if t.shape[-1] % 4 != 0 or t.data_ptr() % 16 != 0 or not t.is_contiguous():
@@ -472,7 +476,7 @@
 class _Linear(torch.autograd.Function):
 
     @staticmethod
-    def forward(ctx, x, w, b, act, unit=False):
+    def forward(ctx, x, w, b, act, unit=False, x_ext=None, arm_out=False):
         x = _req(x.contiguous(), "x"); _req(w, "weight")
         K = x.shape[-1]
         N = w.shape[0]
@@ -482,18 +486,21 @@
         slots = None
         ctx.w_slot = None
         if (ctx.prec & _lib.M3T_GEMM_F16X3) and M % 128 == 0 and N % 64 == 0 and K % 32 == 0 and w.is_contiguous():
-            slots = amax_slots(3, x.device)
+            slots = amax_slots(4, x.device)
             ctx.w_keep = []
             ctx.w_slot = weight_amax(w, ctx.w_keep)
-            ctx.x_slot = amax_one(x.device) if unit else slots.data_ptr()
-            todo = ([] if unit else [(x, slots.data_ptr())]) + ([] if ctx.w_slot is not None else [(w, slots.data_ptr() + 8)])
+            have_x = unit or x_ext is not None
+            ctx.x_slot = amax_one(x.device) if unit else (x_ext.data_ptr() if x_ext is not None else slots.data_ptr())
+            todo = ([] if have_x else [(x, slots.data_ptr())]) + ([] if ctx.w_slot is not None else [(w, slots.data_ptr() + 8)])
             if todo and not measure_amax(todo):
                 slots = None
             elif ctx.w_slot is None:
                 ctx.w_slot = slots.data_ptr() + 8
+        y_slot = slots[3:4] if (arm_out and slots is not None) else None
         sgemm(0, 1, M, N, K, x, 0, K, w, 0, K, y, 0, N, bias=b, act=act, prec=ctx.prec, exclusive=True,
-              amax=(None, None) if slots is None else (ctx.x_slot, ctx.w_slot))
-        ctx.save_for_backward(x, w, y if act else None, slots)
+              amax=(None, None) if slots is None else (ctx.x_slot, ctx.w_slot), amax_c=_p(y_slot))
+        _OUT_SLOT[0] = y_slot
+        ctx.save_for_backward(x, w, y if act else None, slots, x_ext if (slots is not None and not unit) else None)
         ctx.act, ctx.has_bias = act, b is not None
         ctx.bias_ref = b if (b is not None and id(b) in _GRAD_SINKS) else None
         ctx.weight_ref = w if id(w) in _GRAD_SINKS else None
@@ -501,15 +508,20 @@
 
     @staticmethod
     def backward(ctx, dy):
-        x, w, y, slots = ctx.saved_tensors
+        x, w, y, slots, _x_ext = ctx.saved_tensors
+        g_slot = _grad_slot(dy)[0] if slots is not None else None
         dy = _req(dy.contiguous(), "dy")
+        dy_armed = False
         if ctx.act:
-            dy = mask_pos(y, dy)
+            dy = mask_pos(y, dy, amax=slots.data_ptr() + 16 if slots is not None else None)
+            dy_armed, g_slot = slots is not None, None
         K, N = x.shape[-1], w.shape[0]
         M = x.numel() // K
         dx = dw = db = None
         a_x = a_w = a_dy = None
-        if slots is not None and measure_amax([(dy, slots.data_ptr() + 16)]):
+        if g_slot is not None:
+            a_x, a_w, a_dy = ctx.x_slot, ctx.w_slot, g_slot.data_ptr()
+        elif slots is not None and (dy_armed or measure_amax([(dy, slots.data_ptr() + 16)])):
             a_x, a_w, a_dy = ctx.x_slot, ctx.w_slot, slots.data_ptr() + 16
         if ctx.needs_input_grad[0]:
             dx = torch.empty_like(x)
@@ -529,6 +541,8 @@
                     sgemm(1, 0, N, K, M, dy, 0, N, x, 0, K, w_sink, 0, K, prec=ctx.prec, amax=(a_dy, a_x))
                     if slots is not None:
                         slots.record_stream(wg)
+                    if g_slot is not None:
+                        g_slot.record_stream(wg)
             else:
                 dw = w_sink if w_sink is not None else torch.empty_like(w)
                 sgemm(1, 0, N, K, M, dy, 0, N, x, 0, K, dw, 0, K, prec=ctx.prec, exclusive=True, amax=(a_dy, a_x))
@@ -548,7 +562,7 @@
             x.record_stream(wg)
             _WGRAD_PENDING[(x.device.type, x.device.index)] = True
             _LINEAR_RR[0] += 1
-        return dx, dw, db, None, None
+        return dx, dw, db, None, None, None, None
 
 
 _LINEAR_RR = [0]
@@ -640,8 +654,10 @@
     return _ReluDropout.apply(y, float(p), int(seed))
 
 
-def linear(x, w, b=None, act=0):
-    return _Linear.apply(x, w, b, act, _is_unit(x))
+def linear(x, w, b=None, act=0, arm_out=False):
+    x_ext = _tagged_slot(x)
+    _OUT_SLOT[0] = None
+    return _tag_out(_Linear.apply(x, w, b, act, _is_unit(x), x_ext, bool(arm_out)))
 
 
 SCAN_PER_STEP = [False]
@@ -963,9 +979,13 @@
         prec = _PREC[0]
         groups = _stream_groups(Hs, B)
         fslots = None
+        x_ext, ctx.dx_share = _MB_SIDE[0], _MB_SIDE[1]
+        _MB_SIDE[0] = _MB_SIDE[1] = None
+        x_ext = {s: t for s, t in enumerate(x_ext or []) if t is not None and not (unit_mask >> s) & 1}
+        ctx.x_ext = x_ext
         if (prec & _lib.M3T_GEMM_F16X3) and all(h % 4 == 0 for h in Hs):
             fslots = amax_slots(n_stacks * (1 + 2 * L), dev)
-            items = [(xs[s], fslots.data_ptr() + 8 * s) for s in range(n_stacks) if not (unit_mask >> s) & 1]
+            items = [(xs[s], fslots.data_ptr() + 8 * s) for s in range(n_stacks) if not (unit_mask >> s) & 1 and s not in x_ext]
             wslot = {}
             ctx.w_keep = []
             for l in range(L):
@@ -981,6 +1001,8 @@
         one = amax_one(dev)
 
         def fslot_x(l, s):
+            if fslots is not None and l == 0 and s in x_ext:
+                return x_ext[s].data_ptr()
             return None if fslots is None else (fslots.data_ptr() + 8 * s if (l == 0 and not (unit_mask >> s) & 1) else one)
 
         def fslot_w(l, s, d):
@@ -1231,6 +1253,14 @@
         wht = [[[None if direct_whh else new(Hs[s], 3 * Hs[s]) for _ in (0, 1)] for s in range(n_stacks)] for _ in range(L)]
         need_dx = [[l > 0 or ctx.needs_input_grad[5 + s * per] for s in range(n_stacks)] for l in range(L)]
         dinp = [[torch.empty_like(layer_io(l, s)[0]) if need_dx[l][s] else None for s in range(n_stacks)] for l in range(L)]
+        dx_into = {}
+        if ctx.dx_share is not None:
+            for s, t in enumerate(ctx.dx_share.pop("dx", None) or []):
+                if s < n_stacks and t is not None and need_dx[0][s]:
+                    if t.shape != xs[s].shape or not t.is_contiguous():
+                        raise M3THipError("multi_bigru: the dx hand-over of stack %d does not match its input" % s)
+                    dx_into[s] = dinp[0][s] = t
+        dx_slots = amax_slots(n_stacks, dev) if dx_into else None
         for s in range(n_stacks):
             for l in range(L):
                 for d in (0, 1):
@@ -1255,12 +1285,16 @@
             return None if bslots is None else bslots.data_ptr() + 8 * (((l * n_stacks + s) * 2 + d) * NSL + 1 + j)
 
         def fslot_x(l, s):
+            if fslots is not None and l == 0 and s in ctx.x_ext:
+                return ctx.x_ext[s].data_ptr()
             return None if fslots is None else (fslots.data_ptr() + 8 * s if (l == 0 and not (ctx.unit_mask >> s) & 1) else one)
 
         def fslot_w(l, s, d):
             return None if fslots is None else ctx.wslot[(l, s, d)]
 
         def chunk_plan(l, idxs):
+            if l == 0 and dx_into:
+                return None
             if bslots is None or len({Hs[i] for i in idxs}) != 1 or 2 * len(idxs) > M3T_MAX_SCANS or not any(need_dx[l][s] for s in idxs):
                 return None
             H = Hs[idxs[0]]
@@ -1372,9 +1406,14 @@
                 inp, out, gts = layer_io(l, s)
                 I = inp.shape[-1]
                 if need_dx[l][s]:
+                    into = l == 0 and s in dx_into
+                    arm = into and bslots is not None and I % 4 == 0
                     for d in (0, 1):
                         sgemm(0, 0, B * T, I, 3 * H, dgx[l][s], d * 3 * H, 6 * H, params[s][(2 * l + d) * 4], 0, I,
-                              dinp[l][s], 0, I, accumulate=(d == 1), prec=prec, amax=(bslot(l, s, d), fslot_w(l, s, d)))
+                              dinp[l][s], 0, I, accumulate=(d == 1 or into), prec=prec, amax=(bslot(l, s, d), fslot_w(l, s, d)),
+                              amax_c=dx_slots.data_ptr() + 8 * s if (arm and d == 1) else None)
+                    if arm:
+                        _note_grad_slot(dinp[l][s], dx_slots[s:s + 1])
                     cur[s] = dinp[l][s]
 
         wgs = wgrad_streams(dev)
@@ -1506,7 +1545,7 @@
                     for t in (dgx[l][s], dgh[l][s]) + tuple(layer_io(l, s)[:2]):
                         for w_ in wgs:
                             t.record_stream(w_)
-            for t in (bslots, fslots):
+            for t in (bslots, fslots) + tuple(ctx.x_ext.values()):
                 if t is not None:
                     for w_ in wgs:
                         t.record_stream(w_)
@@ -1519,7 +1558,10 @@
         return (None, None, None, None, None) + tuple(None if sunk[i] else g for i, g in enumerate(out_grads))
 
 
-def multi_bigru(stacks, cat=None):
+_MB_SIDE = [None, None]
+
+
+def multi_bigru(stacks, cat=None, dx_share=None):
     L = stacks[0][2]
     flat = []
     for x, prm, l in stacks:
@@ -1529,7 +1571,12 @@
         flat.extend(prm)
     lo, hi = cat if cat is not None else (0, 0)
     unit_mask = sum(1 << i for i, (x, _, _) in enumerate(stacks) if _is_unit(x))
-    res = _MultiBiGRU.apply(len(stacks), L, lo, hi, unit_mask, *flat)
+    _MB_SIDE[0] = [_tagged_slot(x) for x, _, _ in stacks]
+    _MB_SIDE[1] = dx_share
+    try:
+        res = _MultiBiGRU.apply(len(stacks), L, lo, hi, unit_mask, *flat)
+    finally:
+        _MB_SIDE[0] = _MB_SIDE[1] = None
     for i in range(len(stacks)):
         if res[2 * i].numel():
             res[2 * i]._m3t_unit = res[2 * i]._version + 1
@@ -1568,6 +1615,88 @@
 
 def att_fuse(s_v, s_a, x_v, x_a):
     return _AttFuse.apply(s_v, s_a, x_v, x_a)
+
+
+ATT_BLOCK = [os.environ.get("M3T_ATT_BLOCK", "1") != "0"]
+
+
+class _AttFuseScored(torch.autograd.Function):
+
+    @staticmethod
+    def forward(ctx, o_v, o_a, w_v, b_v, w_a, b_a, x_v, x_a, share):
+        o_v, o_a = _req(o_v.contiguous(), "o_v"), _req(o_a.contiguous(), "o_a")
+        x_v, x_a = _req(x_v.contiguous(), "x_v"), _req(x_a.contiguous(), "x_a")
+        D, S = x_v.shape[-1], o_v.shape[-1]
+        rows = x_v.numel() // D
+        for w in (w_v, w_a):
+            if _req(w, "head weight").numel() != S:
+                raise M3THipError("att_fuse_scored: a head must be Linear(%d, 1)" % S)
+        if x_a.shape != x_v.shape or o_a.shape != o_v.shape or o_v.numel() != rows * S:
+            raise M3THipError("att_fuse_scored: shape mismatch")
+        f = torch.empty_like(x_v)
+        s_v = torch.empty(rows, dtype=torch.float32, device=x_v.device)
+        s_a = torch.empty_like(s_v)
+        slot = amax_slots(1, x_v.device) if (_PREC[0] & _lib.M3T_GEMM_F16X3) else None
+        with _Timed("att_fuse_fwd_kernel", 1, 0, nbytes=4.0 * rows * (3 * D + 2 * S + 2)):
+            _armed_call(_p(slot), "m3t_att_fuse_scored_fwd", _p(o_v), _p(o_a), _p(w_v), _p(w_a), _p(b_v), _p(b_a), _p(x_v), _p(x_a), _p(f),
+                        _p(s_v), _p(s_a), rows, D, S, _stream())
+        _OUT_SLOT[0] = slot
+        ctx.save_for_backward(o_v, o_a, w_v, w_a, s_v, s_a, x_v, x_a)
+        ctx.has_bias = (b_v is not None, b_a is not None)
+        ctx.refs = [p if (p is not None and id(p) in _GRAD_SINKS) else None for p in (w_v, b_v, w_a, b_a)]
+        ctx.share = share if (share is not None and ctx.needs_input_grad[0] and ctx.needs_input_grad[1]) else None
+        return f
+
+    @staticmethod
+    def backward(ctx, df):
+        o_v, o_a, w_v, w_a, s_v, s_a, x_v, x_a = ctx.saved_tensors
+        df = _req(df.contiguous(), "df")
+        D, S = x_v.shape[-1], o_v.shape[-1]
+        rows = x_v.numel() // D
+        ds_v, ds_a = torch.empty_like(s_v), torch.empty_like(s_a)
+        dx_v, dx_a = torch.empty_like(x_v), torch.empty_like(x_a)
+        do_v, do_a = torch.empty_like(o_v), torch.empty_like(o_a)
+        with _Timed("att_fuse_bwd_kernel", 1, 0, nbytes=4.0 * rows * (5 * D + 2 * S + 4)):
+            _lib.check(lib().m3t_att_fuse_scored_bwd(_p(df), _p(s_v), _p(s_a), _p(x_v), _p(x_a), _p(w_v), _p(w_a), _p(ds_v), _p(ds_a),
+                                                     _p(dx_v), _p(dx_a), _p(do_v), _p(do_a), rows, D, S, _stream()), "m3t_att_fuse_scored_bwd")
+        need = ctx.needs_input_grad
+        want = [need[2], ctx.has_bias[0] and need[3], need[4], ctx.has_bias[1] and need[5]]
+        sinks = [(_take_sink(r) if (r is not None and want[i]) else None) for i, r in enumerate(ctx.refs)]
+        if any(want[i] and ctx.refs[i] is not None and sinks[i] is None for i in range(4)):
+            join_wgrad(x_v.device)
+        wg = wgrad_stream(x_v.device, _LINEAR_RR[0]) if x_v.is_cuda else None
+        sunk = wg is not None and any(s_ is not None for s_ in sinks)
+        if sunk:
+            wg.wait_stream(cur_stream())
+        grads = [None] * 4
+        for h, (ds, o, w) in enumerate(((ds_v, o_v, w_v), (ds_a, o_a, w_a))):
+            for j in (0, 1):
+                i = 2 * h + j
+                if not want[i]:
+                    continue
+                off = sinks[i] is not None and wg is not None
+                dst = sinks[i] if sinks[i] is not None else torch.empty(S if j == 0 else 1, dtype=torch.float32, device=x_v.device)
+                with (on_stream(wg) if off else _NULL):
+                    if j == 0:
+                        sgemm(1, 0, 1, S, rows, ds, 0, 1, o, 0, S, dst, 0, S, prec=_PREC[0], exclusive=not off)
+                    else:
+                        colsum(ds, 0, rows, 1, 1, dst)
+                if sinks[i] is None:
+                    grads[i] = dst.view(1, S) if j == 0 else dst
+        if sunk:
+            for t in (ds_v, ds_a, o_v, o_a):
+                t.record_stream(wg)
+            _WGRAD_PENDING[(x_v.device.type, x_v.device.index)] = True
+            _LINEAR_RR[0] += 1
+        if ctx.share is not None:
+            ctx.share["dx"] = [dx_v if need[6] else None, dx_a if need[7] else None]
+            dx_v = dx_a = None
+        return do_v, do_a, grads[0], grads[1], grads[2], grads[3], dx_v, dx_a, None
+
+
+def att_fuse_scored(o_v, o_a, fc_v, fc_a, x_v, x_a, share=None):
+    _OUT_SLOT[0] = None
+    return _tag_out(_AttFuseScored.apply(o_v, o_a, fc_v.weight, fc_v.bias, fc_a.weight, fc_a.bias, x_v, x_a, share))
 
 
 class _VALoss(torch.autograd.Function):
diff --git a/m3f.pytorch_amd/m3t/workloads.py b/m3f.pytorch_amd/m3t/workloads.py
--- a/m3f.pytorch_amd/m3t/workloads.py
+++ b/m3f.pytorch_amd/m3t/workloads.py
@@ -23,7 +23,7 @@
 
     def forward(self, x_a, x_v):
         a, v12 = run_grus_cat([self.audio, self.visual.gru_v, self.visual.gru_a], [x_a, x_v, x_v], 1, 3)
-        v = ops.linear(v12, self.proj_v.weight, self.proj_v.bias, 0)
+        v = ops.linear(v12, self.proj_v.weight, self.proj_v.bias, 0, arm_out=ops.ATT_BLOCK[0])
         return self.fusion(self.att_fuse(a, v))
 
 
diff --git a/m3f.pytorch_amd/models/att_fusion.py b/m3f.pytorch_amd/models/att_fusion.py
--- a/m3f.pytorch_amd/models/att_fusion.py
+++ b/m3f.pytorch_amd/models/att_fusion.py
@@ -14,7 +14,17 @@
         self.scorer_a = GRU(d_audio, hidden_dim, 1, 1, 1)
         self.scorer_v = GRU(d_audio, hidden_dim, 1, 1, 1)
 
+    def _one_block(self):
+        def plain(m):
+            return (m.num_layers == 1 and isinstance(getattr(m, "fc", None), nn.Linear) and m.fc.out_features == 1
+                    and m.fc.in_features == 2 * m.hidden_size)
+        return ops.ATT_BLOCK[0] and not self.use_proj and plain(self.scorer_v) and plain(self.scorer_a)
+
     def forward(self, x_a, x_v):
+        if self._one_block():
+            share = {}
+            (o_v, _), (o_a, _) = ops.multi_bigru([self.scorer_v.stack(x_v), self.scorer_a.stack(x_a)], dx_share=share)
+            return ops.att_fuse_scored(o_v, o_a, self.scorer_v.fc, self.scorer_a.fc, x_v, x_a, share)
         if self.use_proj:
             x_v = ops.linear(x_v, self.proj_v.weight, self.proj_v.bias, 0)
         s_v, s_a = run_grus([self.scorer_v, self.scorer_a], [x_v, x_a])
```

Measured after the change: 2859, median of 6. About the same (+0.4%).
